# zhen6618/EPRecon

Hardware: AMD Instinct MI355X
Metric: fragments_per_sec (higher is better)
Workload: dtype f32

## Files before the change

### eprecon_amd/_lib.py

```python
import ctypes
import os

import torch

_HERE = os.path.dirname(os.path.abspath(__file__))
LIB_PATH = os.environ.get("EPRECON_LIB_PATH") or os.path.join(_HERE, "libeprecon_hip.so")

_c = ctypes
_vp, _i, _i64, _f, _sz = _c.c_void_p, _c.c_int, _c.c_int64, _c.c_float, _c.c_size_t

SIGNATURES = {
    "eprecon_abi_version": (_i, []),
    "eprecon_build_arch": (_c.c_char_p, []),
    "eprecon_back_project_workspace_bytes": (_sz, [_i64, _i, _i, _i, _i, _i, _i]),
    "eprecon_back_project_async": (_i, [_vp, _i64, _vp, _i, _f, _vp, _i, _vp, _i, _i, _i, _i, _i, _i,
                                        _vp, _vp, _vp, _vp, _vp, _vp, _vp, _vp, _sz, _vp]),
    "eprecon_back_project": (_i, [_vp, _i64, _vp, _i, _f, _vp, _i, _vp, _i, _i, _i, _i, _i, _i, _i,
                                  _vp, _vp, _vp, _vp, _vp, _vp, _vp, _vp, _vp, _sz, _vp]),
    "eprecon_profile_gather_kernel": (_c.c_char_p, []),
    "eprecon_hash_capacity": (_c.c_uint32, [_i64]),
    "eprecon_hash_table_bytes": (_sz, [_c.c_uint32]),
    "eprecon_hash_build_async": (_i, [_vp, _i64, _i, _vp, _c.c_uint32, _vp]),
    "eprecon_hash_build_dn_async": (_i, [_vp, _i64, _vp, _i, _vp, _c.c_uint32, _vp]),
    "eprecon_hash_query_async": (_i, [_vp, _c.c_uint32, _vp, _i64, _i, _vp, _vp]),
    "eprecon_hash_status": (_i, [_vp, _vp]),
    "eprecon_unique_workspace_bytes": (_sz, [_i64]),
    "eprecon_unique_coords_async": (_i, [_vp, _i64, _i, _vp, _c.c_uint32, _vp, _vp, _vp, _vp, _sz, _vp]),
    "eprecon_unique_coords_dn_async": (_i, [_vp, _i64, _vp, _i, _vp, _c.c_uint32, _vp, _vp, _vp, _vp, _sz, _vp]),
    "eprecon_unique_hierarchy_dn_async": (_i, [_vp, _i64, _vp, _i, _vp, _vp, _vp, _vp, _vp, _vp, _sz, _vp]),
    "eprecon_point_quantize_dn_async": (_i, [_vp, _i64, _vp, _f, _vp, _vp, _vp]),
    "eprecon_spvcnn_points_dn_async": (_i, [_vp, _i64, _vp, _i, _i, _vp, _i, _f, _vp, _f, _vp, _vp, _vp, _vp, _vp, _vp]),
    "eprecon_gru_stage_capacity": (_i64, [_vp, _i64, _i]),
    "eprecon_gru_stage_workspace_bytes": (_sz, [_i64]),
    "eprecon_gru_stage_begin_async": (_i, [_vp, _vp]),
    "eprecon_gru_stage_commit_async": (_i, [_vp, _vp, _vp, _vp]),
    "eprecon_kernel_map_async": (_i, [_vp, _c.c_uint32, _vp, _i64, _i, _i, _vp, _vp]),
    "eprecon_kernel_map_self_async": (_i, [_vp, _c.c_uint32, _vp, _i64, _i, _vp, _vp]),
    "eprecon_transpose_map_async": (_i, [_vp, _i64, _vp, _i, _vp, _vp]),
    "eprecon_sparse_conv_async": (_i, [_vp, _i64, _i, _vp, _i, _i64, _vp, _i, _i, _vp, _vp, _i, _i, _i, _vp]),
    "eprecon_conv_bn_partial_bytes": (_sz, [_i64, _i]),
    "eprecon_sparse_conv_fused_async": (_i, [_vp, _i64, _i, _vp, _i, _i64, _vp, _i, _i, _vp, _vp, _i, _vp, _i, _i, _i,
                                             _vp, _vp]),
    "eprecon_conv_desc_async": (_i, [_vp, _vp]),
    "eprecon_exclusive_scan_async": (_i, [_vp, _i64, _vp, _vp, _vp, _vp]),
    "eprecon_conv_desc_partial_rows": (_i64, [_vp]),
    "eprecon_bn_acc_words": (_sz, [_i]),
    "eprecon_conv_desc_takes_bn_acc": (_i, [_vp]),
    "eprecon_batchnorm_acc_affine_async": (_i, [_vp, _i, _i, _i, _f, _vp, _vp, _vp]),
    "eprecon_affine_rows_acc_async": (_i, [_vp, _i64, _i, _i, _vp, _i, _i, _f, _i, _vp, _i, _vp]),
    "eprecon_affine_rows_res_async": (_i, [_vp, _i64, _i, _i, _vp, _vp, _vp, _i, _i, _vp, _i, _vp]),
    "eprecon_batchnorm_finalize_affine_async": (_i, [_vp, _i64, _i, _vp, _vp, _f, _vp, _vp, _vp]),
    "eprecon_affine_rows_async": (_i, [_vp, _i64, _i, _i, _vp, _vp, _i, _vp, _i, _vp]),
    "eprecon_pixel_map_async": (_i, [_i, _i, _i, _i, _vp, _vp]),
    "eprecon_batchnorm_apply_workspace_bytes": (_sz, [_i]),
    "eprecon_batchnorm_apply_partials_async": (_i, [_vp, _i64, _i, _i, _vp, _i64, _vp, _vp, _f, _vp, _i, _i, _vp, _i,
                                                    _vp, _vp, _vp, _sz, _vp]),
    "eprecon_batchnorm_apply_partials_res_async": (_i, [_vp, _i64, _i, _i, _vp, _i64, _vp, _vp, _f, _vp, _i, _vp, _vp, _i, _vp,
                                                        _i, _vp, _sz, _vp]),
    "eprecon_batchnorm_workspace_bytes": (_sz, [_i64, _i]),
    "eprecon_batchnorm_train_async": (_i, [_vp, _i64, _i, _i, _vp, _vp, _f, _vp, _i, _i, _vp, _i, _vp, _vp,
                                           _vp, _sz, _vp]),
    "eprecon_rowwise_layernorm_async": (_i, [_vp, _i64, _i, _i, _vp, _i, _vp, _vp, _f, _i, _i, _vp, _i, _vp]),
    "eprecon_init_select_workspace_bytes": (_sz, [_i, _i]),
    "eprecon_init_select_async": (_i, [_vp, _vp, _i64, _f, _i, _i, _i, _vp, _vp, _vp, _sz, _vp]),
    "eprecon_upsample_async": (_i, [_vp, _i, _vp, _i64, _i, _i, _vp, _vp, _vp]),
    "eprecon_aligned_coords_async": (_i, [_vp, _i64, _vp, _i, _f, _vp, _vp, _vp]),
    "eprecon_point_quantize_async": (_i, [_vp, _i64, _f, _vp, _vp, _vp]),
    "eprecon_segment_workspace_bytes": (_sz, [_i64, _i64]),
    "eprecon_segment_lists_async": (_i, [_vp, _i64, _i64, _vp, _vp, _vp, _sz, _vp]),
    "eprecon_segment_mean_async": (_i, [_vp, _i, _vp, _vp, _i64, _i, _vp, _i, _vp]),
    "eprecon_sphash_async": (_i, [_vp, _i64, _vp, _vp]),
    "eprecon_sphash_order_workspace_bytes": (_sz, [_i64]),
    "eprecon_sphash_order_async": (_i, [_vp, _i64, _vp, _vp, _vp, _sz, _vp]),
    "eprecon_remap_index_async": (_i, [_vp, _i64, _vp, _vp, _i64, _vp, _vp]),
    "eprecon_trilinear_map_async": (_i, [_vp, _c.c_uint32, _vp, _i64, _i, _vp, _vp, _vp]),
    "eprecon_devoxelize_async": (_i, [_vp, _i, _vp, _vp, _i64, _i, _vp, _i, _i, _vp]),
    "eprecon_sparse_conv_wgrad_workspace_bytes": (_sz, [_i, _i64, _i, _i]),
    "eprecon_sparse_conv_wgrad_async": (_i, [_vp, _i, _vp, _i, _vp, _i, _i64, _i, _i, _vp, _vp, _sz, _vp]),
    "eprecon_invert_map_async": (_i, [_vp, _i, _i64, _i64, _vp, _vp]),
    "eprecon_devoxelize_backward_async": (_i, [_vp, _i, _vp, _vp, _i64, _i, _i64, _vp, _i, _vp]),
    "eprecon_gather_rows_scaled_async": (_i, [_vp, _i, _vp, _vp, _i64, _i, _vp, _i, _vp]),
    "eprecon_back_project_backward_async": (_i, [_vp, _i64, _vp, _i, _f, _vp, _vp, _i, _i, _i, _i, _i, _vp, _i, _vp, _vp, _vp]),
    "eprecon_back_project_backward_workspace_bytes": (_sz, [_i, _i, _i, _i, _i]),
    "eprecon_back_project_backward_det_async": (_i, [_vp, _i64, _vp, _i, _f, _vp, _vp, _i, _i, _i, _i, _i, _vp, _i, _vp, _vp, _vp, _sz,
                                                     _vp]),
    "eprecon_devoxelize_backward_csr_async": (_i, [_vp, _i, _vp, _vp, _vp, _i64, _i, _vp, _i, _vp]),
    "eprecon_devoxelize_gate_async": (_i, [_vp, _i, _vp, _vp, _i64, _i, _vp, _i, _i, _vp, _i, _vp, _i, _vp, _i, _vp]),
    "eprecon_devoxelize_gate_tail_async": (_i, [_vp, _i, _vp, _vp, _i64, _i, _vp, _i, _i, _vp, _i, _vp, _i, _vp, _i, _vp, _i, _vp, _i,
                                                _i, _vp]),
    "eprecon_fbv_union_workspace_bytes": (_sz, [_i]),
    "eprecon_fbv_union_async": (_i, [_vp, _vp, _i64, _i, _vp, _vp, _i64, _i, _i, _i, _i, _i, _vp, _vp, _vp, _vp, _vp,
                                     _vp, _vp, _sz, _vp]),
    "eprecon_map_set_fragment": (_i, [_vp, _i]),
    "eprecon_map_stamps_async": (_i, [_vp, _vp, _vp, _i, _c.c_int32, _vp]),
    "eprecon_map_select_boundary_async": (_i, [_vp, _vp, _i, _i, _i, _vp, _vp]),
    "eprecon_map_pack_boundary_async": (_i, [_vp, _vp, _i64, _vp]),
    "eprecon_map_merge_boundary": (_i, [_vp, _vp, _i64, _vp, _i, _vp, _vp]),
    "eprecon_map_create": (_i, [_i, _c.POINTER(_vp)]),
    "eprecon_map_destroy": (_i, [_vp]),
    "eprecon_map_reset": (_i, [_vp]),
    "eprecon_map_size": (_i64, [_vp]),
    "eprecon_map_channels": (_i, [_vp]),
    "eprecon_map_export_async": (_i, [_vp, _vp, _vp, _vp]),
    "eprecon_map_import_async": (_i, [_vp, _vp, _vp, _i64, _vp]),
    "eprecon_map_crop_union": (_i, [_vp, _vp, _vp, _i64, _i, _i, _i, _i, _vp, _vp, _vp, _vp, _vp, _vp]),
    "eprecon_map_gather_async": (_i, [_vp, _vp, _i64, _i, _i, _f, _vp, _i, _vp]),
    "eprecon_map_update_async": (_i, [_vp, _vp, _i64, _vp, _i, _vp]),
    "eprecon_map_target_fuse": (_i, [_vp, _vp, _vp, _i, _vp, _vp, _i64, _vp, _vp]),
    "eprecon_gather_rows_async": (_i, [_vp, _i, _vp, _i64, _i, _f, _vp, _i, _vp]),
    "eprecon_tsdf_integrate_async": (_i, [_vp, _vp, _vp, _vp, _f, _vp, _i, _i, _i, _vp, _vp, _f, _f, _i, _vp, _vp]),
    "eprecon_marching_cubes_table": (_i, [_vp]),
    "eprecon_marching_cubes_workspace_bytes": (_sz, [_i, _i, _i]),
    "eprecon_marching_cubes_count": (_i, [_vp, _i, _i, _i, _f, _vp, _vp, _sz, _vp]),
    "eprecon_marching_cubes_emit_async": (_i, [_vp, _i, _i, _i, _f, _vp, _vp, _vp, _vp, _vp, _vp, _vp, _vp, _vp]),
    "eprecon_marching_cubes_count_masked": (_i, [_vp, _vp, _i, _i, _i, _f, _vp, _vp, _sz, _vp]),
    "eprecon_marching_cubes_emit_masked_async": (_i, [_vp, _vp, _i, _i, _i, _f, _vp, _vp, _vp, _vp, _vp, _vp, _vp, _vp, _vp]),
    "eprecon_render_depth_workspace_bytes": (_sz, [_i64]),
    "eprecon_render_depth_async": (_i, [_vp, _i64, _vp, _i64, _vp, _i, _i, _i, _f, _f, _f, _i, _vp, _i64, _vp, _sz, _vp]),
    "eprecon_depth_metrics_workspace_bytes": (_sz, [_i]),
    "eprecon_depth_metrics_async": (_i, [_vp, _vp, _i, _i64, _vp, _vp, _sz, _vp]),
    "eprecon_point_bounds_async": (_i, [_vp, _i64, _vp, _vp, _vp]),
    "eprecon_voxel_down_sample_workspace_bytes": (_sz, [_i64, _i64]),
    "eprecon_voxel_down_sample": (_i, [_vp, _i64, _vp, _c.c_double, _vp, _vp, _vp, _i64, _vp, _sz, _vp]),
    "eprecon_nn_search_workspace_bytes": (_sz, [_i64, _i64]),
    "eprecon_nn_search_async": (_i, [_vp, _i64, _vp, _i64, _vp, _c.c_double, _vp, _vp, _vp, _vp, _sz, _vp]),
    "eprecon_nearest_voxel_async": (_i, [_vp, _c.c_uint32, _vp, _i64, _vp, _i64, _i, _vp, _vp]),
    "eprecon_upsample2x_nhwc_async": (_i, [_vp, _vp, _i, _i, _i, _i, _vp]),
    "eprecon_decoder_keys_async": (_i, [_vp, _i, _vp, _i, _vp, _vp, _vp, _i64, _i, _vp, _vp, _vp]),
    "eprecon_decoder_query_side_async": (_i, [_vp, _vp]),
    "eprecon_panoptic_stats_async": (_i, [_vp, _i64, _vp, _vp, _i, _i64, _vp, _vp, _vp, _vp]),
    "eprecon_panoptic_assign_async": (_i, [_vp, _vp, _vp, _i64, _vp, _vp]),
    "eprecon_masked_attention_workspace_bytes": (_sz, [_i64, _i, _i, _i]),
    "eprecon_masked_attention_async": (_i, [_vp, _i, _i, _vp, _i, _vp, _i, _i64, _vp, _i, _vp, _i64, _i, _i, _i, _f, _vp, _vp, _sz, _vp]),
    "eprecon_profile_enable": (_i, [_i]),
    "eprecon_profile_gather_ms": (_f, []),
    "eprecon_profile_conv_arm": (_i, [_i, _i, _i, _i64]),
    "eprecon_profile_conv_ms": (_f, [_c.POINTER(_i64), _c.POINTER(_c.c_char_p)]),
    "eprecon_profile_conv_pairs": (_i64, []),
    "eprecon_mlp4x_supported": (_i, [_i, _i]),
    "eprecon_spvcnn_forward_workspace_bytes": (_sz, [_vp]),
    "eprecon_spvcnn_forward_async": (_i, [_vp, _vp]),
# ... 14 lines not shown
    "eprecon_sparsify_workspace_bytes": (_sz, [_i64]),
    "eprecon_sparsify_async": (_i, [_vp, _i, _f, _vp, _vp, _vp, _i, _vp, _i, _i, _i, _i64, _i, _vp, _vp, _vp, _vp, _vp, _vp, _vp,
                                    _sz, _vp]),
    "eprecon_grid_rank_async": (_i, [_vp, _i64, _i, _i, _i, _i, _vp, _vp]),
    "eprecon_conv_pack_weight_floats": (_sz, [_i, _i, _i]),
    "eprecon_conv_pack_weight_async": (_i, [_vp, _i, _i, _i, _vp, _vp]),
    "eprecon_conv_pack_weight16_floats": (_sz, [_i, _i, _i]),
    "eprecon_conv_pack_weight16_async": (_i, [_vp, _i, _i, _i, _vp, _vp]),
    "eprecon_conv_pack_many_async": (_i, [_vp, _i, _vp]),
    "eprecon_nchw_to_nhwc_async": (_i, [_vp, _vp, _i, _i, _i, _vp]),
    "eprecon_views_to_rows_async": (_i, [_vp, _vp]),
}

EPRECON_OK, EPRECON_EMPTY = 0, 1
ABI_VERSION = 1


class EpreconError(RuntimeError):
    pass


_lib = None


def load():
    global _lib
    if _lib is not None:
        return _lib
    if not os.path.exists(LIB_PATH):
        raise EpreconError(
            f"{LIB_PATH} not found: build it with `python -m eprecon_amd.build` "
            "(hipcc --offload-arch=gfx950). eprecon_amd has no CPU fallback.")
    lib = ctypes.CDLL(LIB_PATH)
    for name, (res, args) in SIGNATURES.items():
        fn = getattr(lib, name)
        fn.restype = res
        fn.argtypes = args
    if lib.eprecon_abi_version() != ABI_VERSION:
        raise EpreconError("libeprecon_hip.so ABI version mismatch; rebuild")
    _lib = lib
    return lib


def check(rc, what):
    if rc == EPRECON_OK:
        return True
    if rc == EPRECON_EMPTY:
        return False
    if rc <= -1000:
        raise EpreconError(f"{what}: HIP error {-(rc + 1000)}")
    raise EpreconError(f"{what}: error {rc} "
                       "(-1 bad argument, -2 workspace too small, -3 unsupported size)")


def ptr(t):
    return None if t is None else t.data_ptr()


_raw_stream = getattr(torch._C, "_cuda_getCurrentRawStream", None)
_raw_device = getattr(torch._C, "_cuda_getDevice", None)


def current_stream():
    if _raw_stream is not None and _raw_device is not None:
        return _raw_stream(_raw_device()) or None
    return torch.cuda.current_stream().cuda_stream or None


class ViewsDesc(ctypes.Structure):
    _fields_ = [("src", (ctypes.c_void_p * 16) * 3), ("dst", ctypes.c_void_p * 3), ("channels", ctypes.c_int32 * 3),
                ("hw", ctypes.c_int32 * 3), ("levels", ctypes.c_int32), ("n_views", ctypes.c_int32)]


class ConvDesc(ctypes.Structure):
    _fields_ = [("x", ctypes.c_void_p), ("n_in", ctypes.c_int64), ("ld_x", ctypes.c_int),
                ("nbr", ctypes.c_void_p), ("kvol", ctypes.c_int), ("n_out", ctypes.c_int64),
                ("weight", ctypes.c_void_p), ("cin", ctypes.c_int), ("cout", ctypes.c_int),
                ("bias", ctypes.c_void_p),
                ("residual", ctypes.c_void_p), ("ld_res", ctypes.c_int),
                ("out", ctypes.c_void_p), ("ld_out", ctypes.c_int),
                ("relu", ctypes.c_int), ("accumulate", ctypes.c_int),
                ("in_scale", ctypes.c_void_p), ("in_shift", ctypes.c_void_p), ("in_relu", ctypes.c_int),
                ("res_scale", ctypes.c_void_p), ("res_shift", ctypes.c_void_p), ("res_relu", ctypes.c_int),
                ("bn_partial", ctypes.c_void_p),
                ("ln", ctypes.c_int), ("ln_gamma", ctypes.c_void_p), ("ln_beta", ctypes.c_void_p),
                ("ln_eps", ctypes.c_float), ("ln_post_relu", ctypes.c_int),
                ("img_h", ctypes.c_int), ("img_w", ctypes.c_int), ("img_maps", ctypes.c_int),
                ("vox_rank", ctypes.c_void_p), ("grid_x", ctypes.c_int), ("grid_y", ctypes.c_int), ("grid_z", ctypes.c_int),
                ("packed_weight", ctypes.c_void_p), ("packed_weight16", ctypes.c_void_p),
                ("workspace", ctypes.c_void_p), ("workspace_bytes", ctypes.c_size_t),
                ("bn_acc", ctypes.c_void_p), ("bn_acc_ld", ctypes.c_int), ("bn_acc_c0", ctypes.c_int),
                ("bn_gamma", ctypes.c_void_p), ("bn_beta", ctypes.c_void_p),
                ("in_acc", ctypes.c_void_p), ("in_acc_ld", ctypes.c_int), ("in_acc_c0", ctypes.c_int),
                ("in_eps", ctypes.c_float), ("in_affine_scratch", ctypes.c_void_p)]


class GruStageDesc(ctypes.Structure):
    _fields_ = [("map", ctypes.c_void_p), ("target_map", ctypes.c_void_p),
                ("cur_coords", ctypes.c_void_p), ("cur_feat", ctypes.c_void_p), ("n_cur", ctypes.c_int64), ("ld_cur", ctypes.c_int),
                ("dim", ctypes.c_int), ("interval", ctypes.c_int), ("activity_mode", ctypes.c_int),
                ("rel", ctypes.c_int32 * 3),
                ("tsdf_gt", ctypes.c_void_p), ("occ_gt", ctypes.c_void_p),
                ("origin", ctypes.c_void_p), ("w2ac", ctypes.c_void_p),
                ("voxel_size", ctypes.c_float), ("resolution", ctypes.c_float),
                ("ch_voxel", ctypes.c_int), ("batch_index", ctypes.c_int),
                ("capacity", ctypes.c_int64),
                ("updated", ctypes.c_void_p), ("out_coords", ctypes.c_void_p), ("r_coords", ctypes.c_void_p),
                ("hx_voxel", ctypes.c_void_p), ("hx_image", ctypes.c_void_p), ("tsdf_target", ctypes.c_void_p),
                ("scaled1", ctypes.c_void_p), ("vox1", ctypes.c_void_p), ("inverse1", ctypes.c_void_p), ("uniq1", ctypes.c_void_p),
                ("table1", ctypes.c_void_p),
                ("scaled2", ctypes.c_void_p), ("vox2", ctypes.c_void_p), ("inverse2", ctypes.c_void_p), ("uniq2", ctypes.c_void_p),
                ("table2", ctypes.c_void_p),
                ("table_capacity", ctypes.c_uint32),
                ("counts", ctypes.c_void_p),
                ("workspace", ctypes.c_void_p), ("workspace_bytes", ctypes.c_size_t)]


class DecoderLayerDesc(ctypes.Structure):
    _PTRS_A = ["o_attn", "state_in", "query_pos", "cross_out_wt", "cross_out_b", "cross_ln_g", "cross_ln_b", "self_in_wt", "self_in_b",
               "self_out_wt", "self_out_b", "self_ln_g", "self_ln_b", "ffn1_wt", "ffn1_b", "ffn2_wt", "ffn2_b", "ffn_ln_g", "ffn_ln_b",
               "dec_ln_g", "dec_ln_b", "cls_wt", "cls_b", "m1_wt", "m1_b", "m2_wt", "m2_b", "m3_wt", "m3_b", "next_q_wt", "next_q_b"]
    _PTRS_B = ["state_out", "cls_out", "mask_embed_out", "next_q_out", "workspace"]
    _fields_ = ([(n, ctypes.c_int) for n in ("n_queries", "channels", "n_heads", "ffn_dim", "n_class_logits", "mask_hidden")]
                + [(n, ctypes.c_void_p) for n in _PTRS_A] + [("ln_eps", ctypes.c_float)] + [(n, ctypes.c_void_p) for n in _PTRS_B])


class GruFinishDesc(ctypes.Structure):
    _fields_ = ([(n, ctypes.c_int64) for n in ("n", "m1", "m2")]
                + [(n, ctypes.c_void_p) for n in ("inverse1", "inverse2", "uniq1", "uniq2", "table1", "table2")]
                + [("table_capacity", ctypes.c_uint32)] + [(n, ctypes.c_void_p) for n in ("scaled1", "scaled2")]
                + [("literal", ctypes.c_int)]
                + [(n, ctypes.c_void_p) for n in ("offsets1", "order1", "offsets2", "order2", "nbr1", "nbr2", "idx8_1", "weight8_1",
                                                  "idx8_2", "weight8_2", "perm1", "rank1", "perm2", "rank2", "workspace")]
                + [("workspace_bytes", ctypes.c_size_t)])


class SpvcnnGeometryDesc(ctypes.Structure):
    _fields_ = ([(n, ctypes.c_int64) for n in ("n", "n1", "n2", "n4")]
                + [(n, ctypes.c_void_p) for n in ("scaled", "vox", "inverse1", "coords1", "coords2", "coords4", "parent2", "parent4",
                                                  "table1", "table2", "table4")]
                + [(n, ctypes.c_uint32) for n in ("capacity1", "capacity2", "capacity4")]
                + [(n, ctypes.c_void_p) for n in ("offsets1", "order1", "idx4", "offsets4", "order4", "down12", "up21", "down24", "up42",
                                                  "k1", "k2", "k4", "idx8_1", "weight8_1", "idx8_4", "weight8_4", "workspace")]
                + [("workspace_bytes", ctypes.c_size_t)])


SPVCNN_CONVS = 27


class SpvcnnConv(ctypes.Structure):
    _fields_ = [(n, ctypes.c_void_p) for n in ("weight", "packed_weight", "packed_weight16")] + [(n, ctypes.c_int) for n in ("kvol", "cin", "cout")]


class SpvcnnBn(ctypes.Structure):
    _fields_ = [("gamma", ctypes.c_void_p), ("beta", ctypes.c_void_p), ("eps", ctypes.c_float)]


class SpvcnnForwardDesc(ctypes.Structure):
    _fields_ = ([(n, ctypes.c_int64) for n in ("n", "n1", "n2", "n4")] + [("cin", ctypes.c_int), ("cs", ctypes.c_int * 5)]
                + [("feat", ctypes.c_void_p), ("ld_feat", ctypes.c_int)]
                + [(n, ctypes.c_void_p) for n in ("offsets1", "order1", "offsets4", "order4", "k1", "k2", "k4", "down12", "up21", "down24",
                                                  "up42", "idx8_1", "weight8_1", "idx8_4", "weight8_4")]
                + [("conv", SpvcnnConv * SPVCNN_CONVS), ("bn", SpvcnnBn * SPVCNN_CONVS)]
                + [("out", ctypes.c_void_p), ("ld_out", ctypes.c_int), ("workspace", ctypes.c_void_p), ("workspace_bytes", ctypes.c_size_t)])


class Mlp4xHead(ctypes.Structure):
# ... 129 lines not shown
```

### eprecon_amd/csrc/conv_common.hpp

```cpp
#pragma once
#include "common.hpp"

namespace epconv {

struct ConvParams {
    const float *x;
    const int32_t *nbr;
    const float *w;
    const float *bias;
    float *out;
    int n_out, K, Cin, Cout, ld_x, ld_out;
    int64_t x_bytes;
    int relu;
    int accumulate;
    const float *res;
    int ld_res;
    float *bn_partial;
    const float *in_scale, *in_shift;
    int in_relu;
    const float *res_scale, *res_shift;
    int res_relu;
    int ln;
    const float *ln_gamma, *ln_beta;
    float ln_eps;
    int ln_post_relu;
    int img_h, img_w, img_maps;
    int flex_partial;
    const int32_t *vox_rank;
    int gx, gy, gz;
    const float *wq;
    const float *wq16;
    int debug;
    int splitk_pipe;
    void *ws;
    size_t ws_bytes;
    long long *bn_acc;
    int bn_acc_ld, bn_acc_c0;
    const float *bn_gamma, *bn_beta;
    const long long *in_acc;
    int in_acc_ld, in_acc_c0;
    float in_eps;
};

constexpr int kBnCopies = 8, kBnWords = 7;
#ifndef EP_BN_ABL
#define EP_BN_ABL 0
#endif

__device__ __forceinline__ void bn_limbs(double x, long long &l0, long long &l1, long long &l2)
{
    const double v = x * 1099511627776.0;
    const double hi = floor(v * (1.0 / 1099511627776.0));
    l0 = (long long)(v - hi * 1099511627776.0);
    const long long h = (long long)hi;
    l1 = h & ((1ll << 40) - 1);
    l2 = h >> 40;
}

__device__ __forceinline__ void bn_acc_add(long long *acc, int ld, int c, int copy, float n, float mean, float m2)
{
    if (n <= 0.0f || (EP_BN_ABL & 1)) return;
    unsigned long long *a = reinterpret_cast<unsigned long long *>(acc) + ((size_t)copy * ld + c) * kBnWords;
    const double dn = (double)n, dm = (double)mean;
    long long l0, l1, l2;
    bn_limbs(dn * dm, l0, l1, l2);
    atomicAdd(a + 0, (unsigned long long)l0);
    if (EP_BN_ABL & 4) return;
    atomicAdd(a + 1, (unsigned long long)l1); atomicAdd(a + 2, (unsigned long long)l2);
    bn_limbs((double)m2 + dn * dm * dm, l0, l1, l2);
    atomicAdd(a + 3, (unsigned long long)l0); atomicAdd(a + 4, (unsigned long long)l1); atomicAdd(a + 5, (unsigned long long)l2);
    atomicAdd(a + 6, (unsigned long long)(long long)n);
}

__device__ __forceinline__ void bn_acc_affine(const long long *acc, int ld, int c, float eps, float &scale, float &shift)
{
    if (EP_BN_ABL & 2) { scale = 1.0f; shift = 0.0f; return; }
    long long w[kBnWords] = {0, 0, 0, 0, 0, 0, 0};
#pragma unroll 1
    for (int k = 0; k < kBnCopies; ++k) {
        const long long *a = acc + ((size_t)k * ld + c) * kBnWords;
#pragma unroll
        for (int j = 0; j < kBnWords; ++j) w[j] += a[j];
    }
    const double two40 = 1099511627776.0;
    const double s1 = ((double)w[2] * two40 + (double)w[1]) + (double)w[0] * (1.0 / two40);
    const double s2 = ((double)w[5] * two40 + (double)w[4]) + (double)w[3] * (1.0 / two40);
    const double n = (double)w[6];
    const float *gb = reinterpret_cast<const float *>(acc + (size_t)kBnCopies * ld * kBnWords);
    const double mean = n > 0.0 ? s1 / n : 0.0;
    double var = n > 0.0 ? s2 / n - mean * mean : 0.0;
    if (var < 0.0) var = 0.0;
    const float sc = gb[c] / sqrtf((float)var + eps);
    scale = sc;
    shift = gb[ld + c] - (float)mean * sc;
}

template <int THREADS, bool ACC = true>
__device__ __forceinline__ void stage_in_affine(const ConvParams &p, float *sAff, int cpad, int tid)
{
    if (!p.in_scale) return;
    for (int c = tid; c < cpad; c += THREADS) {
        float sc = 0.0f, sh = 0.0f;
        if (c < p.Cin) {
            if (ACC && p.in_acc) bn_acc_affine(p.in_acc, p.in_acc_ld, p.in_acc_c0 + c, p.in_eps, sc, sh);
            else { sc = p.in_scale[c]; sh = p.in_shift[c]; }
        }
        sAff[c] = sc;
        sAff[cpad + c] = sh;
    }
}

__device__ __forceinline__ void bn_acc_publish(const ConvParams &p, int col, int copy, bool first, float n, float mean, float m2)
{
    bn_acc_add(p.bn_acc, p.bn_acc_ld, p.bn_acc_c0 + col, copy & (kBnCopies - 1), n, mean, m2);
    if (first) {
        float *gb = reinterpret_cast<float *>(p.bn_acc + (size_t)kBnCopies * p.bn_acc_ld * kBnWords);
        gb[p.bn_acc_c0 + col] = p.bn_gamma ? p.bn_gamma[col] : 1.0f;
        gb[p.bn_acc_ld + p.bn_acc_c0 + col] = p.bn_beta ? p.bn_beta[col] : 0.0f;
    }
}

constexpr int kWaves = 4;
typedef float f32x4 __attribute__((ext_vector_type(4)));
typedef unsigned int u32x4 __attribute__((ext_vector_type(4)));

__device__ __forceinline__ void chan_merge(float &n_a, float &mean_a, float &m2_a, float n_b, float mean_b, float m2_b)
{
    if (n_b == 0.0f) return;
    if (n_a == 0.0f) {
        n_a = n_b; mean_a = mean_b; m2_a = m2_b;
        return;
    }
    const float n = n_a + n_b;
    const float d = mean_b - mean_a;
    mean_a = mean_a + d * (n_b / n);
    m2_a = m2_a + m2_b + d * d * (n_a * n_b / n);
    n_a = n;
}

template <int CT, bool ACC = false>
__device__ __forceinline__ void tile16_epilogue(const ConvParams &p, const f32x4 (&acc)[CT], const int (&orow)[4], float *sStat,
                                                int partial_row)
{
    const int tid = threadIdx.x;
    const int lane = tid & 63, wave = tid >> 6;
    const int l16 = lane & 15, q = lane >> 4;
    float v[CT][4];
    bool colok[CT];
#pragma unroll
    for (int t = 0; t < CT; ++t) {
        const int col = 16 * t + l16;
        colok[t] = col < p.Cout;
        const float b = (p.bias && colok[t]) ? p.bias[col] : 0.0f;
        const float rs = (p.res_scale && colok[t]) ? p.res_scale[col] : 1.0f;
        const float rb = (p.res_scale && colok[t]) ? p.res_shift[col] : 0.0f;
#pragma unroll
        for (int j = 0; j < 4; ++j) {
            float val = 0.0f;
            if (colok[t] && orow[j] >= 0) {
                val = acc[t][j] + b;
                if (p.relu) val = fmaxf(val, 0.0f);
                if (p.res) {
                    float rv = p.res[(size_t)orow[j] * p.ld_res + col];
                    if (p.res_scale) {
                        rv = fmaf(rv, rs, rb);
                        if (p.res_relu) rv = fmaxf(rv, 0.0f);
                    }
                    val += rv;
                }
            }
            v[t][j] = val;
        }
    }
    if (p.ln) {
        const float inv_c = 1.0f / (float)p.Cout;
#pragma unroll
        for (int j = 0; j < 4; ++j) {
            float sum = 0.0f;
#pragma unroll
            for (int t = 0; t < CT; ++t) sum += v[t][j];
#pragma unroll
            for (int m = 8; m > 0; m >>= 1) sum += __shfl_xor(sum, m);
            const float mean = sum * inv_c;
            float sq = 0.0f;
#pragma unroll
            for (int t = 0; t < CT; ++t) {
                const float d = colok[t] ? v[t][j] - mean : 0.0f;
                v[t][j] = d;
                sq = fmaf(d, d, sq);
            }
#pragma unroll
            for (int m = 8; m > 0; m >>= 1) sq += __shfl_xor(sq, m);
            const float inv = 1.0f / sqrtf(sq * inv_c + p.ln_eps);
#pragma unroll
            for (int t = 0; t < CT; ++t) {
                const int col = 16 * t + l16;
                float y = fmaf(v[t][j] * inv, (p.ln_gamma && colok[t]) ? p.ln_gamma[col] : 1.0f, (p.ln_beta && colok[t]) ? p.ln_beta[col] : 0.0f);
                if (p.ln_post_relu) y = fmaxf(y, 0.0f);
                v[t][j] = y;
            }
        }
    }
#pragma unroll
    for (int t = 0; t < CT; ++t)
#pragma unroll
        for (int j = 0; j < 4; ++j)
            if (colok[t] && orow[j] >= 0) p.out[(size_t)orow[j] * p.ld_out + 16 * t + l16] = v[t][j];
    if (p.bn_partial || (ACC && p.bn_acc)) {
#pragma unroll
        for (int t = 0; t < CT; ++t) {
            float n = 0.0f, sum = 0.0f;
#pragma unroll
            for (int j = 0; j < 4; ++j)
                if (orow[j] >= 0) { n += 1.0f; sum += v[t][j]; }
            float mean = n > 0.0f ? sum / n : 0.0f, m2 = 0.0f;
#pragma unroll
            for (int j = 0; j < 4; ++j)
                if (orow[j] >= 0) { const float d = v[t][j] - mean; m2 = fmaf(d, d, m2); }
#pragma unroll
            for (int m = 16; m < 64; m <<= 1) {
                const float on = __shfl_xor(n, m), om = __shfl_xor(mean, m), oq = __shfl_xor(m2, m);
                const bool lower = (lane & m) == 0;
                float a_n = lower ? n : on, a_mean = lower ? mean : om, a_m2 = lower ? m2 : oq;
                chan_merge(a_n, a_mean, a_m2, lower ? on : n, lower ? om : mean, lower ? oq : m2);
                n = a_n; mean = a_mean; m2 = a_m2;
            }
            if (q == 0) {
                float *d = sStat + (wave * 3) * 16 * CT + 16 * t + l16;
                d[0] = n; d[16 * CT] = mean; d[2 * 16 * CT] = m2;
            }
        }
        __syncthreads();
        if (tid < 16 * CT && tid < p.Cout) {
            float a_n = 0.0f, a_mean = 0.0f, a_m2 = 0.0f;
#pragma unroll
            for (int w = 0; w < kWaves; ++w)
                chan_merge(a_n, a_mean, a_m2, sStat[(w * 3) * 16 * CT + tid], sStat[(w * 3 + 1) * 16 * CT + tid], sStat[(w * 3 + 2) * 16 * CT + tid]);
            if (p.bn_partial) {
                float *dst = p.bn_partial + (size_t)partial_row * 3 * p.Cout + tid;
                dst[0] = a_n; dst[p.Cout] = a_mean; dst[2 * p.Cout] = a_m2;
            }
            if (ACC && p.bn_acc) bn_acc_publish(p, tid, partial_row, partial_row == 0, a_n, a_mean, a_m2);
        }
    }
}

bool direct16_ok(const ConvParams &p);
constexpr int kDirectRows = 128;
int launch_direct16(const ConvParams &p, hipStream_t st);
int direct16_partial_block_rows(const ConvParams &p);

bool tile2d16_ok(const ConvParams &p);
int64_t tile2d16_partial_rows(const ConvParams &p);
int launch_tile2d16(const ConvParams &p, hipStream_t st);


}
```

### eprecon_amd/csrc/norm.hip

```cpp
#include <stdlib.h>

#include "common.hpp"
#include "conv_common.hpp"

namespace {
using namespace ep;

constexpr int kBnPerThread = 8;

__device__ __forceinline__ void chan_merge(float &n_a, float &mean_a, float &m2_a, float n_b, float mean_b, float m2_b)
{
    if (n_b == 0.0f) return;
    if (n_a == 0.0f) {
        n_a = n_b; mean_a = mean_b; m2_a = m2_b;
        return;
    }
    const float n = n_a + n_b;
    const float d = mean_b - mean_a;
    mean_a = mean_a + d * (n_b / n);
    m2_a = m2_a + m2_b + d * d * (n_a * n_b / n);
    n_a = n;
}

__global__ __launch_bounds__(256) void bn_stats_kernel(const float *x, int n, int C, int ld, float *partial)
{
    __shared__ float sN[256], sMean[256], sM2[256];
    const int tid = threadIdx.x;
    const int rpi = 256 / C;
    const int col = tid % C, rsub = tid / C;
    const bool active = rsub < rpi;
    const int r0 = blockIdx.x * (kBnPerThread * rpi);
    float v[kBnPerThread];
    float cnt = 0.0f, sum = 0.0f;
#pragma unroll
    for (int k = 0; k < kBnPerThread; ++k) {
        const int r = r0 + k * rpi + rsub;
        const bool ok = active && r < n;
        v[k] = ok ? x[(size_t)r * ld + col] : 0.0f;
        cnt += ok ? 1.0f : 0.0f;
        sum += v[k];
    }
    const float mean = cnt > 0.0f ? sum / cnt : 0.0f;
    float m2 = 0.0f;
#pragma unroll
    for (int k = 0; k < kBnPerThread; ++k) {
        const int r = r0 + k * rpi + rsub;
        if (active && r < n) {
            const float d = v[k] - mean;
            m2 = fmaf(d, d, m2);
        }
    }
    sN[tid] = cnt; sMean[tid] = mean; sM2[tid] = m2;
    __syncthreads();
    for (int s = 1; s < rpi; s <<= 1) {
        if (active && (rsub % (2 * s)) == 0 && rsub + s < rpi) {
            float n = sN[tid], m = sMean[tid], q = sM2[tid];
            const int o = tid + s * C;
            chan_merge(n, m, q, sN[o], sMean[o], sM2[o]);
            sN[tid] = n; sMean[tid] = m; sM2[tid] = q;
        }
        __syncthreads();
    }
    if (tid < C) {
        float *p = partial + (size_t)blockIdx.x * 3 * C;
        p[tid] = sN[tid]; p[C + tid] = sMean[tid]; p[2 * C + tid] = sM2[tid];
    }
}

__global__ __launch_bounds__(256) void bn_finalize_kernel(const float *partial, int nblk, int C, float *mean_out,
                                                          float *var_out)
{
    __shared__ float sN[256], sMean[256], sM2[256];
    const int c = blockIdx.x, tid = threadIdx.x;
    float a_n = 0.0f, a_mean = 0.0f, a_m2 = 0.0f;
    for (int b = tid; b < nblk; b += 4 * 256) {
        float vn[4], vm[4], vq[4];
#pragma unroll
        for (int u = 0; u < 4; ++u) {
            const int bb = b + u * 256;
            const float *p = partial + (size_t)(bb < nblk ? bb : b) * 3 * C;
            vn[u] = bb < nblk ? p[c] : 0.0f;
            vm[u] = p[C + c];
            vq[u] = p[2 * C + c];
        }
#pragma unroll
        for (int u = 0; u < 4; ++u) chan_merge(a_n, a_mean, a_m2, vn[u], vm[u], vq[u]);
    }
    sN[tid] = a_n; sMean[tid] = a_mean; sM2[tid] = a_m2;
    __syncthreads();
    for (int s = 128; s > 0; s >>= 1) {
        if (tid < s) {
            float n = sN[tid], m = sMean[tid], q = sM2[tid];
            chan_merge(n, m, q, sN[tid + s], sMean[tid + s], sM2[tid + s]);
            sN[tid] = n; sMean[tid] = m; sM2[tid] = q;
        }
        __syncthreads();
    }
    if (tid == 0) {
        mean_out[c] = sMean[0];
        var_out[c] = sN[0] > 0.0f ? sM2[0] / sN[0] : 0.0f;
    }
}

__global__ __launch_bounds__(256) void bn_finalize_affine_kernel(const float *partial, int nblk, int C, const float *gamma,
                                                                 const float *beta, float eps, float *scale_out,
                                                                 float *shift_out)
{
    __shared__ float sN[4], sMean[4], sM2[4];
    const int c = blockIdx.x, tid = threadIdx.x;
    const float g_c = gamma ? gamma[c] : 1.0f, b_c = beta ? beta[c] : 0.0f;
    float a_n = 0.0f, a_mean = 0.0f, a_m2 = 0.0f;
    for (int b = tid; b < nblk; b += 4 * 256) {
        float vn[4], vm[4], vq[4];
#pragma unroll
        for (int u = 0; u < 4; ++u) {
            const int bb = b + u * 256;
            const float *p = partial + (size_t)(bb < nblk ? bb : b) * 3 * C;
            vn[u] = bb < nblk ? p[c] : 0.0f;
            vm[u] = p[C + c];
            vq[u] = p[2 * C + c];
        }
#pragma unroll
        for (int u = 0; u < 4; ++u) chan_merge(a_n, a_mean, a_m2, vn[u], vm[u], vq[u]);
    }
    const int lane = tid & 63;
#pragma unroll
    for (int m = 1; m < 64; m <<= 1) {
        const float on = __shfl_xor(a_n, m), om = __shfl_xor(a_mean, m), oq = __shfl_xor(a_m2, m);
        float ln = (lane & m) ? on : a_n, lm = (lane & m) ? om : a_mean, lq = (lane & m) ? oq : a_m2;
        chan_merge(ln, lm, lq, (lane & m) ? a_n : on, (lane & m) ? a_mean : om, (lane & m) ? a_m2 : oq);
        a_n = ln; a_mean = lm; a_m2 = lq;
    }
    if (lane == 0) { sN[tid >> 6] = a_n; sMean[tid >> 6] = a_mean; sM2[tid >> 6] = a_m2; }
    __syncthreads();
    if (tid == 0) {
        float n = sN[0], mean = sMean[0], m2 = sM2[0];
        for (int w = 1; w < 4; ++w) chan_merge(n, mean, m2, sN[w], sMean[w], sM2[w]);
        const float var = n > 0.0f ? m2 / n : 0.0f;
        const float sc = g_c / sqrtf(var + eps);
        scale_out[c] = sc;
        shift_out[c] = b_c - mean * sc;
    }
}

__global__ __launch_bounds__(256) void bn_apply_kernel(const float *x, int n, int C, int ld_x,
                                                       const float *mean, const float *var,
                                                       const float *gamma, const float *beta, float eps,
                                                       const float *res, int ld_res, const float *res_scale,
                                                       const float *res_shift, int relu, float *out, int ld_out)
{
    const size_t e = (size_t)blockIdx.x * 256 + threadIdx.x;
    if (e >= (size_t)n * C) return;
    const int r = (int)(e / C), c = (int)(e - (size_t)r * C);
    const float inv = 1.0f / sqrtf(var[c] + eps);
    float v = (x[(size_t)r * ld_x + c] - mean[c]) * inv;
    v = v * (gamma ? gamma[c] : 1.0f) + (beta ? beta[c] : 0.0f);
    if (res) {
        float rv = res[(size_t)r * ld_res + c];
        if (res_scale) rv = fmaf(rv, res_scale[c], res_shift[c]);
        v += rv;
    }
    if (relu) v = fmaxf(v, 0.0f);
    out[(size_t)r * ld_out + c] = v;
}

__global__ __launch_bounds__(256) void rowwise_ln_kernel(const float *x, int n, int C, int ld_x,
                                                         const float *res, int ld_res,
                                                         const float *gamma, const float *beta, float eps,
                                                         int pre_relu, int post_relu, float *out,
                                                         int ld_out)
{
    const int g = threadIdx.x & 7;
    const int r = blockIdx.x * 32 + (threadIdx.x >> 3);
    const bool live = r < n;
    const float *xr = x + (size_t)(live ? r : 0) * ld_x;
    const float *rr = res ? res + (size_t)(live ? r : 0) * ld_res : nullptr;
    auto value = [&](int c) -> float {
        float v = xr[c];
        if (pre_relu) v = fmaxf(v, 0.0f);
        if (rr) v += rr[c];
        return v;
    };
    float s = 0.0f;
    if (live)
        for (int c = g; c < C; c += 8) s += value(c);
    s += __shfl_xor(s, 1);
    s += __shfl_xor(s, 2);
    s += __shfl_xor(s, 4);
    const float mean = s / (float)C;
    float q = 0.0f;
    if (live)
        for (int c = g; c < C; c += 8) {
            const float d = value(c) - mean;
            q = fmaf(d, d, q);
        }
    q += __shfl_xor(q, 1);
    q += __shfl_xor(q, 2);
    q += __shfl_xor(q, 4);
    const float inv = 1.0f / sqrtf(q / (float)C + eps);
    if (live)
        for (int c = g; c < C; c += 8) {
            float v = (value(c) - mean) * inv * (gamma ? gamma[c] : 1.0f) + (beta ? beta[c] : 0.0f);
            if (post_relu) v = fmaxf(v, 0.0f);
            out[(size_t)r * ld_out + c] = v;
        }
}

__global__ __launch_bounds__(256) void affine_rows_kernel(const float *x, int n, int C, int ld_x, const float *scale,
                                                          const float *shift, int relu, float *out, int ld_out)
{
    const size_t e = (size_t)blockIdx.x * 256 + threadIdx.x;
    if (e >= (size_t)n * C) return;
    const int r = (int)(e / C), c = (int)(e - (size_t)r * C);
    float v = fmaf(x[(size_t)r * ld_x + c], scale[c], shift[c]);
    if (relu) v = fmaxf(v, 0.0f);
    out[(size_t)r * ld_out + c] = v;
}

__global__ __launch_bounds__(256) void bn_acc_affine_kernel(const long long *acc, int ld, int c0, int C, float eps, float *scale,
                                                            float *shift)
{
    const int c = blockIdx.x * 256 + threadIdx.x;
    if (c >= C) return;
    float sc, sh;
    epconv::bn_acc_affine(acc, ld, c0 + c, eps, sc, sh);
    scale[c] = sc;
    shift[c] = sh;
}

constexpr int kAccRowsMaxC = 512;
__global__ __launch_bounds__(256) void affine_rows_acc_kernel(const float *x, int n, int C, int ld_x, const long long *acc, int ld,
                                                              int c0, float eps, int relu, float *out, int ld_out)
{
    __shared__ float sAff[2 * kAccRowsMaxC];
    for (int c = threadIdx.x; c < C; c += 256) epconv::bn_acc_affine(acc, ld, c0 + c, eps, sAff[c], sAff[kAccRowsMaxC + c]);
    __syncthreads();
    for (int k = 0; k < 16; ++k) {
        const size_t e = ((size_t)blockIdx.x * 16 + k) * 256 + threadIdx.x;
        if (e >= (size_t)n * C) return;
        const int r = (int)(e / C), c = (int)(e - (size_t)r * C);
        float v = fmaf(x[(size_t)r * ld_x + c], sAff[c], sAff[kAccRowsMaxC + c]);
        if (relu) v = fmaxf(v, 0.0f);
        out[(size_t)r * ld_out + c] = v;
    }
}

__global__ __launch_bounds__(256) void affine_rows_res_kernel(const float *x, int n, int C, int ld_x, const float *scale,
                                                              const float *shift, const float *res, int ld_res, int relu,
                                                              float *out, int ld_out)
{
    const size_t e = (size_t)blockIdx.x * 256 + threadIdx.x;
    if (e >= (size_t)n * C) return;
    const int r = (int)(e / C), c = (int)(e - (size_t)r * C);
    float v = fmaf(x[(size_t)r * ld_x + c], scale[c], shift[c]);
    if (res) v += res[(size_t)r * ld_res + c];
    if (relu) v = fmaxf(v, 0.0f);
    out[(size_t)r * ld_out + c] = v;
}

int bn_finalize_apply(const float *x, int64_t n, int channels, int ld_x, const float *partial, int nblk,
                      const float *gamma, const float *beta, float eps, const float *residual, int ld_res,
                      int relu, float *out, int ld_out, float *mean, float *var, hipStream_t st,
                      const float *res_scale = nullptr, const float *res_shift = nullptr)
{
    hipLaunchKernelGGL(bn_finalize_kernel, dim3(channels), dim3(256), 0, st, partial, nblk, channels, mean, var);
    EP_LAUNCH_CHECK();
    const size_t total = (size_t)n * channels;
    hipLaunchKernelGGL(bn_apply_kernel, dim3((unsigned)ceil_div((int64_t)total, 256)), dim3(256), 0, st, x,
                       (int)n, channels, ld_x, (const float *)mean, (const float *)var, gamma, beta, eps,
                       residual, ld_res, res_scale, res_shift, relu, out, ld_out);
    EP_LAUNCH_CHECK();
    return EPRECON_OK;
}

}

extern "C" {

static inline int bn_rows_per_block(int channels) { return kBnPerThread * (256 / channels); }

size_t eprecon_batchnorm_workspace_bytes(int64_t n, int channels)
{
    if (channels <= 0 || channels > 256) return 0;
    const size_t nblk = (size_t)ceil_div(n > 0 ? n : 1, bn_rows_per_block(channels));
    return align_up(nblk * 3 * channels * sizeof(float), 256) + 2 * align_up((size_t)channels * sizeof(float), 256);
}

int eprecon_batchnorm_train_async(const float *x, int64_t n, int channels, int ld_x, const float *gamma,
                                  const float *beta, float eps, const float *residual, int ld_res,
                                  int relu, float *out, int ld_out, float *mean_out, float *var_out,
                                  void *workspace, size_t workspace_bytes, void *stream)
{
    if (!x || !out || n < 0 || channels <= 0 || channels > 256 || ld_x < channels || ld_out < channels ||
        !workspace)
        return EPRECON_ERR_ARG;
    if (workspace_bytes < eprecon_batchnorm_workspace_bytes(n, channels)) return EPRECON_ERR_WORKSPACE;
    if (n == 0) return EPRECON_OK;
    hipStream_t st = (hipStream_t)stream;
    const int nblk = (int)ceil_div(n, bn_rows_per_block(channels));
    char *ws = reinterpret_cast<char *>(workspace);
    float *partial = reinterpret_cast<float *>(ws);
    ws += align_up((size_t)nblk * 3 * channels * sizeof(float), 256);
    float *mean = mean_out ? mean_out : reinterpret_cast<float *>(ws);
    ws += align_up((size_t)channels * sizeof(float), 256);
    float *var = var_out ? var_out : reinterpret_cast<float *>(ws);
    hipLaunchKernelGGL(bn_stats_kernel, dim3(nblk), dim3(256), 0, st, x, (int)n, channels, ld_x, partial);
    EP_LAUNCH_CHECK();
    return bn_finalize_apply(x, n, channels, ld_x, partial, nblk, gamma, beta, eps, residual, ld_res, relu, out,
                             ld_out, mean, var, st);
}

size_t eprecon_batchnorm_apply_workspace_bytes(int channels)
{
    return 2 * align_up((size_t)(channels > 0 ? channels : 1) * sizeof(float), 256);
}

int eprecon_batchnorm_apply_partials_async(const float *x, int64_t n, int channels, int ld_x,
                                           const float *partial, int64_t nblk, const float *gamma,
                                           const float *beta, float eps, const float *residual,
                                           int ld_res, int relu, float *out, int ld_out, float *mean_out,
                                           float *var_out, void *workspace, size_t workspace_bytes,
                                           void *stream)
{
    if (!x || !out || !partial || n < 0 || nblk <= 0 || nblk > 0x7fffffff || channels <= 0 || ld_x < channels ||
        ld_out < channels || !workspace)
        return EPRECON_ERR_ARG;
    if (workspace_bytes < eprecon_batchnorm_apply_workspace_bytes(channels)) return EPRECON_ERR_WORKSPACE;
    if (n == 0) return EPRECON_OK;
    char *ws = reinterpret_cast<char *>(workspace);
    float *mean = mean_out ? mean_out : reinterpret_cast<float *>(ws);
    ws += align_up((size_t)channels * sizeof(float), 256);
    float *var = var_out ? var_out : reinterpret_cast<float *>(ws);
    return bn_finalize_apply(x, n, channels, ld_x, partial, (int)nblk, gamma, beta, eps, residual, ld_res, relu,
                             out, ld_out, mean, var, (hipStream_t)stream);
}

int eprecon_batchnorm_apply_partials_res_async(const float *x, int64_t n, int channels, int ld_x, const float *partial,
                                               int64_t nblk, const float *gamma, const float *beta, float eps,
                                               const float *residual, int ld_res, const float *res_scale,
                                               const float *res_shift, int relu, float *out, int ld_out, void *workspace,
                                               size_t workspace_bytes, void *stream)
{
    if (!x || !out || !partial || !residual || !res_scale || !res_shift || n < 0 || nblk <= 0 || nblk > 0x7fffffff ||
        channels <= 0 || ld_x < channels || ld_out < channels || ld_res < channels || !workspace)
        return EPRECON_ERR_ARG;
    if (workspace_bytes < eprecon_batchnorm_apply_workspace_bytes(channels)) return EPRECON_ERR_WORKSPACE;
    if (n == 0) return EPRECON_OK;
    char *ws = reinterpret_cast<char *>(workspace);
    float *mean = reinterpret_cast<float *>(ws);
    float *var = reinterpret_cast<float *>(ws + align_up((size_t)channels * sizeof(float), 256));
    return bn_finalize_apply(x, n, channels, ld_x, partial, (int)nblk, gamma, beta, eps, residual, ld_res, relu, out, ld_out,
                             mean, var, (hipStream_t)stream, res_scale, res_shift);
}

int eprecon_batchnorm_finalize_affine_async(const float *partial, int64_t nblk, int channels, const float *gamma,
                                            const float *beta, float eps, float *scale_out, float *shift_out,
                                            void *stream)
{
    if (!partial || !scale_out || !shift_out || nblk <= 0 || nblk > 0x7fffffff || channels <= 0) return EPRECON_ERR_ARG;
    hipLaunchKernelGGL(bn_finalize_affine_kernel, dim3(channels), dim3(256), 0, (hipStream_t)stream, partial, (int)nblk,
                       channels, gamma, beta, eps, scale_out, shift_out);
    EP_LAUNCH_CHECK();
    return EPRECON_OK;
}

int eprecon_affine_rows_async(const float *x, int64_t n, int channels, int ld_x, const float *scale,
                              const float *shift, int relu, float *out, int ld_out, void *stream)
{
    if (!x || !out || !scale || !shift || n < 0 || channels <= 0 || ld_x < channels || ld_out < channels ||
        n * channels > 0x7fffffffll * 256)
        return EPRECON_ERR_ARG;
    if (n == 0) return EPRECON_OK;
    hipLaunchKernelGGL(affine_rows_kernel, dim3((unsigned)ceil_div(n * channels, (int64_t)256)), dim3(256), 0,
                       (hipStream_t)stream, x, (int)n, channels, ld_x, scale, shift, relu, out, ld_out);
    EP_LAUNCH_CHECK();
    return EPRECON_OK;
}

int eprecon_batchnorm_acc_affine_async(const long long *acc, int acc_ld, int acc_c0, int channels, float eps, float *scale_out,
                                       float *shift_out, void *stream)
{
    if (!acc || !scale_out || !shift_out || channels <= 0 || acc_c0 < 0 || acc_c0 + channels > acc_ld) return EPRECON_ERR_ARG;
    hipLaunchKernelGGL(bn_acc_affine_kernel, dim3((unsigned)ceil_div(channels, 256)), dim3(256), 0, (hipStream_t)stream, acc, acc_ld,
                       acc_c0, channels, eps, scale_out, shift_out);
    EP_LAUNCH_CHECK();
    return EPRECON_OK;
}

int eprecon_affine_rows_acc_async(const float *x, int64_t n, int channels, int ld_x, const long long *acc, int acc_ld, int acc_c0,
                                  float eps, int relu, float *out, int ld_out, void *stream)
{
    if (!x || !out || !acc || n < 0 || channels <= 0 || channels > kAccRowsMaxC || ld_x < channels || ld_out < channels ||
        acc_c0 < 0 || acc_c0 + channels > acc_ld || n * channels > 0x7fffffffll * 256)
        return EPRECON_ERR_ARG;
    if (n == 0) return EPRECON_OK;
    hipLaunchKernelGGL(affine_rows_acc_kernel, dim3((unsigned)ceil_div(n * channels, (int64_t)4096)), dim3(256), 0,
                       (hipStream_t)stream, x, (int)n, channels, ld_x, acc, acc_ld, acc_c0, eps, relu, out, ld_out);
    EP_LAUNCH_CHECK();
    return EPRECON_OK;
}

int eprecon_affine_rows_res_async(const float *x, int64_t n, int channels, int ld_x, const float *scale,
                                  const float *shift, const float *residual, int ld_res, int relu, float *out,
                                  int ld_out, void *stream)
{
    if (!x || !out || !scale || !shift || n < 0 || channels <= 0 || ld_x < channels || ld_out < channels ||
        (residual && ld_res < channels) || n * channels > 0x7fffffffll * 256)
        return EPRECON_ERR_ARG;
    if (n == 0) return EPRECON_OK;
    hipLaunchKernelGGL(affine_rows_res_kernel, dim3((unsigned)ceil_div(n * channels, (int64_t)256)), dim3(256), 0,
                       (hipStream_t)stream, x, (int)n, channels, ld_x, scale, shift, residual, ld_res, relu, out, ld_out);
    EP_LAUNCH_CHECK();
    return EPRECON_OK;
}

int eprecon_rowwise_layernorm_async(const float *x, int64_t n, int channels, int ld_x,
                                    const float *residual, int ld_res, const float *gamma,
                                    const float *beta, float eps, int pre_relu, int post_relu,
                                    float *out, int ld_out, void *stream)
{
    if (!x || !out || n < 0 || channels <= 0 || ld_x < channels || ld_out < channels) return EPRECON_ERR_ARG;
    if (n == 0) return EPRECON_OK;
    hipLaunchKernelGGL(rowwise_ln_kernel, dim3((unsigned)ceil_div(n, 32)), dim3(256), 0,
                       (hipStream_t)stream, x, (int)n, channels, ld_x, residual, ld_res, gamma, beta, eps,
                       pre_relu, post_relu, out, ld_out);
    EP_LAUNCH_CHECK();
    return EPRECON_OK;
}

}
```

### eprecon_amd/csrc/sparse_conv.hip

```cpp
#include <stdio.h>
#include <stdlib.h>
#include <string.h>

#include "common.hpp"
#include "conv_common.hpp"

namespace {
using namespace ep;
using namespace epconv;

typedef float f32x16 __attribute__((ext_vector_type(16)));


template <int TN>
__device__ __forceinline__ void stage_weights(float *dst, const float *w, int row0, int row_end, int stride,
                                              int ncols, int rows, int tid)
{
    const int total = rows * TN;
    if (stride == TN && ncols >= TN && (reinterpret_cast<uintptr_t>(w) & 15) == 0) {
        const float4 *src = reinterpret_cast<const float4 *>(w + (size_t)row0 * stride);
        float4 *d4 = reinterpret_cast<float4 *>(dst);
        const int valid4 = max(0, min(rows, row_end - row0)) * (TN / 4);
#pragma unroll 4
        for (int e = tid; e < total / 4; e += 256) d4[e] = e < valid4 ? src[min(e, max(valid4 - 1, 0))] : make_float4(0.f, 0.f, 0.f, 0.f);
// ... 93 lines not shown
        const float inv = 1.0f / sqrtf(q * inv_c + p.ln_eps);
        const int row = rm((r & 3) + 8 * (r >> 2) + 4 * half);
#pragma unroll
        for (int t = 0; t < NT; ++t) {
            float y = fmaf(acc[t][r] * inv, gam[t], bet[t]);
            if (p.ln_post_relu) y = fmaxf(y, 0.0f);
            if (colok[t] && row >= 0) p.out[(size_t)row * p.ld_out + t * 32 + r32] = y;
        }
    }
}

template <int NT, bool ACC = true, class RowMap>
__device__ __forceinline__ void conv_epilogue(const ConvParams &p, f32x16 (&acc)[NT], RowMap rm, int col0, int r32,
                                              int half, int wave, float *sStat, int partial_row, int ncb)
{
    constexpr int TN = 32 * NT;
    if (p.ln) {
        conv_epilogue_ln<NT>(p, acc, rm, r32, half);
        return;
    }
    const bool stats = p.bn_partial != nullptr || (ACC && p.bn_acc != nullptr);
    if (stats) __syncthreads();
#pragma unroll
    for (int t = 0; t < NT; ++t) {
        const int col = col0 + t * 32 + r32;
        const bool colok = col < p.Cout;
        const float b = (p.bias && colok) ? p.bias[col] : 0.0f;
        const float rs = (p.res_scale && colok) ? p.res_scale[col] : 1.0f;
        const float rb = (p.res_scale && colok) ? p.res_shift[col] : 0.0f;
        float vals[16];
        float cnt = 0.0f, sum = 0.0f;
#pragma unroll
        for (int r = 0; r < 16; ++r) {
            const int row = rm((r & 3) + 8 * (r >> 2) + 4 * half);
            float v = 0.0f;
            if (colok && row >= 0) {
                float *o = p.out + (size_t)row * p.ld_out + col;
                v = acc[t][r] + b;
                if (p.accumulate) v += *o;
                if (p.relu) v = fmaxf(v, 0.0f);
                if (p.res) {
                    float rv = p.res[(size_t)row * p.ld_res + col];
                    if (p.res_scale) {
                        rv = fmaf(rv, rs, rb);
                        if (p.res_relu) rv = fmaxf(rv, 0.0f);
                    }
                    v += rv;
                }
                *o = v;
                cnt += 1.0f;
            }
            vals[r] = v;
            sum += v;
        }
        if (stats) {
            float mean = cnt > 0.0f ? sum / cnt : 0.0f;
            float m2 = 0.0f;
#pragma unroll
            for (int r = 0; r < 16; ++r) {
                const int row = rm((r & 3) + 8 * (r >> 2) + 4 * half);
                if (row >= 0) {
                    const float d = vals[r] - mean;
                    m2 = fmaf(d, d, m2);
                }
            }
            const float on = __shfl_xor(cnt, 32), omean = __shfl_xor(mean, 32), om2 = __shfl_xor(m2, 32);
            float a_n = half ? on : cnt, a_mean = half ? omean : mean, a_m2 = half ? om2 : m2;
            chan_merge(a_n, a_mean, a_m2, half ? cnt : on, half ? mean : omean, half ? m2 : om2);
            if (half == 0) {
                float *d = sStat + (wave * 3) * TN + t * 32 + r32;
                d[0] = a_n; d[TN] = a_mean; d[2 * TN] = a_m2;
            }
        }
    }
    if (stats) {
        __syncthreads();
        const int tid = threadIdx.x;
        if (tid < TN && col0 + tid < p.Cout) {
            float a_n = 0.0f, a_mean = 0.0f, a_m2 = 0.0f;
#pragma unroll
            for (int w = 0; w < kWaves; ++w)
                chan_merge(a_n, a_mean, a_m2, sStat[(w * 3) * TN + tid], sStat[(w * 3 + 1) * TN + tid],
                           sStat[(w * 3 + 2) * TN + tid]);
            if (!ACC || p.bn_partial) {
                float *dst = p.bn_partial + (size_t)partial_row * 3 * p.Cout + col0 + tid;
                dst[0] = a_n; dst[p.Cout] = a_mean; dst[2 * p.Cout] = a_m2;
            }
            if (ACC && p.bn_acc) bn_acc_publish(p, col0 + tid, partial_row, partial_row == 0, a_n, a_mean, a_m2);
        }
    }
}

template <int NT, bool VEC4>
__global__ __launch_bounds__(256) void spconv_mfma_kernel(ConvParams p)
{
    extern __shared__ __attribute__((aligned(16))) char smem[];
    constexpr int TN = 32 * NT;
    float *sW = reinterpret_cast<float *>(smem);
    int *sNbr = reinterpret_cast<int *>(sW + 2 * kSlabC * TN);
    int *sActive = sNbr + p.K * kRowsPerBlock;
    const int cinA = (p.Cin + 3) & ~3;
    float *sAff = reinterpret_cast<float *>(sActive + ((p.K + 3) & ~3));

    const int tid = threadIdx.x;
    const int lane = tid & 63, wave = tid >> 6;
    const int r32 = lane & 31, half = lane >> 5;
    const int row0 = blockIdx.x * kRowsPerBlock;
    const int col0 = blockIdx.y * TN;

    for (int k = tid; k < p.K; k += 256) sActive[k] = 0;
    stage_in_affine<256>(p, sAff, cinA, tid);
    __syncthreads();
    for (int e = tid; e < p.K * kRowsPerBlock; e += 256) {
        const int k = e / kRowsPerBlock, r = e - k * kRowsPerBlock;
        const int row = row0 + r;
        int j = -1;
        if (row < p.n_out) j = p.nbr ? p.nbr[(size_t)k * p.n_out + row] : row;
        sNbr[e] = j;
        if (j >= 0) sActive[k] = 1;
    }
    __syncthreads();

    f32x16 acc[NT];
#pragma unroll
    for (int t = 0; t < NT; ++t)
#pragma unroll
        for (int r = 0; r < 16; ++r) acc[t][r] = 0.0f;

    const int nslab = (p.Cin + kSlabC - 1) / kSlabC;
    int buf = 0;
    bool have_prev = false;
    for (int k = 0; k < p.K; ++k) {
        if (!sActive[k]) continue;
        const int j = sNbr[k * kRowsPerBlock + wave * kRowsPerWave + r32];
        const float *xrow = p.x + (size_t)(j >= 0 ? j : 0) * p.ld_x;
        const float *wk = p.w + (size_t)k * p.Cin * p.Cout + col0;
        for (int sl = 0; sl < nslab; ++sl) {
            const int c0 = sl * kSlabC;
            float *dstW = sW + buf * kSlabC * TN;
            stage_weights<TN>(dstW, wk, c0, p.Cin, p.Cout, p.Cout - col0, kSlabC, tid);
            float a[4][4];
#pragma unroll
            for (int ch = 0; ch < 4; ++ch) {
                const int c = c0 + ch * 8 + 4 * half;
                if (VEC4) {
                    float4 v = make_float4(0.f, 0.f, 0.f, 0.f);
                    if (j >= 0 && c < p.Cin) v = *reinterpret_cast<const float4 *>(xrow + c);
                    if (p.Cin & 3) {
                        if (c + 1 >= p.Cin) v.y = 0.0f;
                        if (c + 2 >= p.Cin) v.z = 0.0f;
                        if (c + 3 >= p.Cin) v.w = 0.0f;
                    }
                    a[ch][0] = v.x; a[ch][1] = v.y; a[ch][2] = v.z; a[ch][3] = v.w;
                } else {
#pragma unroll
                    for (int s = 0; s < 4; ++s) a[ch][s] = (j >= 0 && c + s < p.Cin) ? xrow[c + s] : 0.0f;
                }
            }
            __syncthreads();
            (void)have_prev;
            const float *srcW = sW + buf * kSlabC * TN;
            const int nch = min(4, (p.Cin - c0 + 7) / 8);
            if (p.in_scale) {
#pragma unroll
                for (int ch = 0; ch < 4; ++ch) {
                    const int c = c0 + ch * 8 + 4 * half;
#pragma unroll
                    for (int s = 0; s < 4; ++s) {
                        const bool ok = j >= 0 && c + s < p.Cin;
                        float v = fmaf(a[ch][s], sAff[min(c + s, cinA - 1)], sAff[cinA + min(c + s, cinA - 1)]);
// ... 498 lines not shown
    const int v = tid % (32 * WV);
    const int own = d3_rank(sX, (((v >> 5) + 1) * kD3HY + ((v >> 3) & 3) + 1) * kD3HZ + (v & 7) + 1, P, cin_pad);
    return __syncthreads_or(own >= 0) != 0;
}

template <int NCH, int WV, int THREADS = 64 * WV>
__device__ __forceinline__ void d3_stage_rows(const ConvParams &p, float *sX, int tid, int dbg, int cbase)
{
    constexpr int cin_pad = NCH * 8, P = cin_pad + 4, C4 = cin_pad / 4;
    constexpr int kThreads = THREADS, kD3Halo = d3_halo(WV);
    constexpr int kItems = kD3Halo * C4;
    constexpr int kIter = (kItems + kThreads - 1) / kThreads;
    float4 hv[kIter];
    int hr[kIter];
    const int last4 = ((p.Cin + 3) & ~3) - 4;
    constexpr bool kFixedGroup = kThreads % C4 == 0;
    float4 sc0 = make_float4(1.f, 1.f, 1.f, 1.f), sh0 = make_float4(0.f, 0.f, 0.f, 0.f);
    if (kFixedGroup && p.in_scale) {
        sc0 = *reinterpret_cast<const float4 *>(p.in_scale + min(cbase + (tid % C4) * 4, last4));
        sh0 = *reinterpret_cast<const float4 *>(p.in_shift + min(cbase + (tid % C4) * 4, last4));
    }
#pragma unroll
    for (int it = 0; it < kIter; ++it) {
        const int e = min(tid + it * kThreads, kItems - 1);
        const int cell = e / C4, c4 = e - cell * C4;
        hr[it] = d3_rank(sX, cell, P, cin_pad);
        if (dbg & 4) hv[it] = make_float4(1.f, 1.f, 1.f, 1.f);
        else hv[it] = *reinterpret_cast<const float4 *>(p.x + (size_t)max(hr[it], 0) * p.ld_x + min(cbase + c4 * 4, last4));
    }
#pragma unroll
    for (int it = 0; it < kIter; ++it) {
        const int e = tid + it * kThreads;
        if (e >= kItems) break;
        const int cell = e / C4, c4 = e - cell * C4;
        const int c = cbase + c4 * 4;
        float4 v4 = hv[it];
        if (p.in_scale) {
            float4 sc = sc0, sh = sh0;
            if (!kFixedGroup) {
                sc = *reinterpret_cast<const float4 *>(p.in_scale + min(c, last4));
                sh = *reinterpret_cast<const float4 *>(p.in_shift + min(c, last4));
            }
            v4.x = fmaf(v4.x, sc.x, sh.x); v4.y = fmaf(v4.y, sc.y, sh.y);
            v4.z = fmaf(v4.z, sc.z, sh.z); v4.w = fmaf(v4.w, sc.w, sh.w);
            if (p.in_relu) {
                v4.x = fmaxf(v4.x, 0.f); v4.y = fmaxf(v4.y, 0.f); v4.z = fmaxf(v4.z, 0.f); v4.w = fmaxf(v4.w, 0.f);
            }
        }
        if (hr[it] < 0 || c >= p.Cin) v4 = make_float4(0.f, 0.f, 0.f, 0.f);
        *reinterpret_cast<float4 *>(sX + cell * P + c4 * 4) = v4;
    }
    __syncthreads();
}

template <int NCH, int WV, int THREADS = 64 * WV>
__device__ __forceinline__ bool d3_stage_halo(const ConvParams &p, int x0, int y0, int z0, float *sX, int tid, int dbg)
{
    if (!d3_stage_ranks<NCH, WV, THREADS>(p, x0, y0, z0, sX, tid)) return false;
    d3_stage_rows<NCH, WV, THREADS>(p, sX, tid, dbg, 0);
    return true;
}

template <int NCH>
__global__ __launch_bounds__(256) void conv3d_tile_narrow_kernel(ConvParams p, int tiles_y, int tiles_z, int ntiles)
{
    constexpr int cin_pad = NCH * 8, P = cin_pad + 4, C4 = cin_pad / 4;
    constexpr int WV = kD3WvNarrow, kD3Halo = d3_halo(WV);
    static_assert(WV == 4, "the cell mapping below covers 128 cells with 256 threads");
    extern __shared__ __attribute__((aligned(16))) char smem[];
    float *sX = reinterpret_cast<float *>(smem);
    float *sWn = sX + kD3Halo * P;
    float *sRed = sWn + 27 * cin_pad;
    const int tid = threadIdx.x;
    const int lane = tid & 63, wave = tid >> 6;
    const int tile = xcd_remap((int)blockIdx.x, (int)gridDim.x);
    if (tile >= ntiles) return;
    int x0, y0, z0;
    d3_tile_origin<WV>(tile, tiles_y, tiles_z, x0, y0, z0);
    for (int e = tid; e < 27 * cin_pad; e += 256) {
        const int k = e / cin_pad, c = e - k * cin_pad;
        sWn[e] = c < p.Cin ? p.w[((size_t)k * p.Cin + c) * p.Cout] : 0.0f;
    }
    if (!d3_stage_halo<NCH, WV>(p, x0, y0, z0, sX, tid, p.debug)) {
        if (p.bn_partial && tid == 0) {
            float *dst = p.bn_partial + (size_t)tile * 3 * p.Cout;
            dst[0] = 0.0f; dst[p.Cout] = 0.0f; dst[2 * p.Cout] = 0.0f;
        }
        return;
    }
    const int v = tid >> 1, part = tid & 1;
    const int cell0 = (((v >> 5) + 1) * kD3HY + ((v >> 3) & 3) + 1) * kD3HZ + (v & 7) + 1;
    const int row = d3_rank(sX, cell0, P, cin_pad);
    float acc = 0.0f;
#pragma unroll
    for (int k = 0; k < 27; ++k) {
        const int dx = k % 3 - 1, dy = (k / 3) % 3 - 1, dz = k / 9 - 1;
        const float *xk = sX + (cell0 + (dx * kD3HY + dy) * kD3HZ + dz) * P;
#pragma unroll
        for (int j = 0; j < C4 / 2; ++j) {
            const int c = (2 * j + part) * 4;
            const float4 a = *reinterpret_cast<const float4 *>(xk + c);
            const float4 w = *reinterpret_cast<const float4 *>(sWn + k * cin_pad + c);
            acc = fmaf(a.x, w.x, acc); acc = fmaf(a.y, w.y, acc); acc = fmaf(a.z, w.z, acc); acc = fmaf(a.w, w.w, acc);
        }
    }
    acc += __shfl_xor(acc, 1);
    float n = 0.0f, mean = 0.0f, m2 = 0.0f;
    if (part == 0 && row >= 0) {
        float *o = p.out + (size_t)row * p.ld_out;
        float val = acc + (p.bias ? p.bias[0] : 0.0f);
        if (p.accumulate) val += *o;
        if (p.relu) val = fmaxf(val, 0.0f);
        if (p.res) {
            float rv = p.res[(size_t)row * p.ld_res];
            if (p.res_scale) {
                rv = fmaf(rv, p.res_scale[0], p.res_shift[0]);
                if (p.res_relu) rv = fmaxf(rv, 0.0f);
            }
            val += rv;
        }
        *o = val;
        n = 1.0f; mean = val;
    }
    if (p.bn_partial) {
#pragma unroll
        for (int m = 1; m < 64; m <<= 1) {
            const float on = __shfl_xor(n, m), omean = __shfl_xor(mean, m), om2 = __shfl_xor(m2, m);
            const bool lower = (lane & m) == 0;
            float a_n = lower ? n : on, a_mean = lower ? mean : omean, a_m2 = lower ? m2 : om2;
            chan_merge(a_n, a_mean, a_m2, lower ? on : n, lower ? omean : mean, lower ? om2 : m2);
            n = a_n; mean = a_mean; m2 = a_m2;
        }
        if (lane == 0) { sRed[wave * 3] = n; sRed[wave * 3 + 1] = mean; sRed[wave * 3 + 2] = m2; }
        __syncthreads();
        if (tid == 0) {
            float a_n = 0.0f, a_mean = 0.0f, a_m2 = 0.0f;
            for (int w = 0; w < kWaves; ++w) chan_merge(a_n, a_mean, a_m2, sRed[w * 3], sRed[w * 3 + 1], sRed[w * 3 + 2]);
            float *dst = p.bn_partial + (size_t)tile * 3 * p.Cout;
            dst[0] = a_n; dst[p.Cout] = a_mean; dst[2 * p.Cout] = a_m2;
        }
    }
}

constexpr int kD16X = 2;
constexpr int kD16Halo = (kD16X + 2) * kD3HY * kD3HZ;

__device__ __forceinline__ void pack_weights16_body(const float *w, int K, int Cin, int Cout, int kch, int ct, float *wq, int first,
                                                    int step)
{
    const int total = K * kch * ct * 256;
    const int rem = Cout - 16 * (ct - 1);
    const int total_tail = (rem >= 1 && rem <= 8) ? K * kch * 128 : 0;
    for (int e = first; e < total_tail; e += step) {
        const int sidx = e & 3, n = (e >> 2) & 3, q = (e >> 4) & 3, cg = (e >> 6) & 1;
        const int r = e >> 7;
        const int kc = r % kch, k = r / kch;
        const bool tail8 = kc == kch - 1 && Cin - 16 * kc <= 8;
        const int c = tail8 ? (sidx < 2 ? 16 * kc + 2 * q + sidx : Cin) : 16 * kc + 4 * q + sidx;
        const int co = 16 * (ct - 1) + 4 * cg + n;
        wq[(size_t)total + e] = (c < Cin && co < Cout) ? w[((size_t)k * Cin + c) * Cout + co] : 0.0f;
    }
    for (int e = first; e < total; e += step) {
        const int sidx = e & 3, col = (e >> 2) & 15, q = (e >> 6) & 3;
        int r = e >> 8;
        const int t = r % ct; r /= ct;
        const int kc = r % kch, k = r / kch;
        const bool tail8 = kc == kch - 1 && Cin - 16 * kc <= 8;
        const int c = tail8 ? (sidx < 2 ? 16 * kc + 2 * q + sidx : Cin) : 16 * kc + 4 * q + sidx;
        const int co = 16 * t + col;
        wq[e] = (c < Cin && co < Cout) ? w[((size_t)k * Cin + c) * Cout + co] : 0.0f;
    }
}
__global__ void pack_weights16_kernel(const float *w, int K, int Cin, int Cout, int kch, int ct, float *wq)
{
    pack_weights16_body(w, K, Cin, Cout, kch, ct, wq, blockIdx.x * blockDim.x + threadIdx.x, gridDim.x * blockDim.x);
}

__global__ void pack_many_kernel(const eprecon_pack_job *jobs)
{
    const eprecon_pack_job j = jobs[blockIdx.y];
    const int first = blockIdx.x * blockDim.x + threadIdx.x, step = gridDim.x * blockDim.x;
    if (j.kind == 0) {
        int nt, ncb;
        d3_columns(j.cout, &nt, &ncb);
        pack_weights_body(j.weight, j.kvol, j.cin, j.cout, (j.cin + 7) / 8, nt, ncb, j.packed, first, step);
    } else {
        pack_weights16_body(j.weight, j.kvol, j.cin, j.cout, (j.cin + 15) / 16, (j.cout + 15) / 16, j.packed, first, step);
    }
}

#ifndef EP_TILE16_MIX
#define EP_TILE16_MIX 1
#endif
template <int CT, int KCH>
__global__ __launch_bounds__(256, 7) void conv3d_tile16_kernel(ConvParams p, int tiles_y, int tiles_z, int ntiles)
{
    constexpr int cin_pad = 16, NCH = 2;
    constexpr int P = cin_pad + 4;
    extern __shared__ __attribute__((aligned(16))) char smem[];
    float *sX = reinterpret_cast<float *>(smem);
    const int tid = threadIdx.x;
    const int lane = tid & 63, wave = tid >> 6;
    const int l16 = lane & 15, q = lane >> 4;
    const int tile = xcd_remap((int)blockIdx.x, (int)gridDim.x);
    if (tile >= ntiles) return;
    int x0, y0, z0;
    d3_tile_origin<kD16X>(tile, tiles_y, tiles_z, x0, y0, z0);
    float *sStat = sX;

    if (!d3_stage_ranks<NCH, kD16X, 256>(p, x0, y0, z0, sX, tid)) {
        if (p.bn_partial && tid < 16 * CT && tid < p.Cout) {
            float *dst = p.bn_partial + (size_t)tile * 3 * p.Cout + tid;
            dst[0] = 0.0f; dst[p.Cout] = 0.0f; dst[2 * p.Cout] = 0.0f;
        }
        return;
    }
    const int wx = wave >> 1, wy = 2 * (wave & 1);
    const int cell_a = ((wx + 1) * kD3HY + wy + (l16 >> 3) + 1) * kD3HZ + (l16 & 7) + 1;
    int orow[4];
#pragma unroll
    for (int j = 0; j < 4; ++j) {
        const int r = 4 * q + j;
        orow[j] = d3_rank(sX, ((wx + 1) * kD3HY + wy + (r >> 3) + 1) * kD3HZ + (r & 7) + 1, P, cin_pad);
    }
    const bool work = __ballot(d3_rank(sX, cell_a, P, cin_pad) >= 0) != 0ull && !(p.debug & 1);

    f32x4 acc[CT];
#pragma unroll
    for (int t = 0; t < CT; ++t) acc[t] = f32x4{0.0f, 0.0f, 0.0f, 0.0f};

    const float *xa = sX + (cell_a - (kD3HY + 1) * kD3HZ - 1) * P + 4 * q;
    constexpr unsigned kStepBytes = CT * 1024u, kOffBytes = KCH * kStepBytes;
    const __amdgpu_buffer_rsrc_t wrsrc =
        __builtin_amdgcn_make_buffer_rsrc(const_cast<float *>(p.wq), 0, (int)(27 * kOffBytes), 0x00020000);
    const unsigned wlane = (unsigned)lane * 16u;
    constexpr int kAheadB = 2;
    for (int pass = 0; pass < KCH; ++pass) {
        if (pass > 0) __syncthreads();
        d3_stage_rows<NCH, kD16X, 256>(p, sX, tid, p.debug, 16 * pass);
        if (!work) continue;
        float4 bq[kAheadB + 1][CT];
        float4 aq[2];
        auto load_b = [&](int k, float4(&dst)[CT]) {
#pragma unroll
            for (int t = 0; t < CT; ++t) {
                const u32x4 v = __builtin_amdgcn_raw_buffer_load_b128(wrsrc, wlane + (unsigned)t * 1024u,
                                                                      (unsigned)((p.debug & 2) ? 0 : k) * kOffBytes + (unsigned)pass * kStepBytes, 0);
                dst[t] = make_float4(__uint_as_float(v.x), __uint_as_float(v.y), __uint_as_float(v.z), __uint_as_float(v.w));
            }
        };
        auto load_a = [&](int k) {
            const int dx = k % 3, dy = (k / 3) % 3, dz = k / 9;
            return *reinterpret_cast<const float4 *>(xa + ((dx * kD3HY + dy) * kD3HZ + dz) * P);
        };
#pragma unroll
        for (int k = 0; k < kAheadB; ++k) load_b(k, bq[k]);
        aq[0] = load_a(0);
#pragma unroll
        for (int k = 0; k < 27; ++k) {
            if (k + kAheadB < 27) load_b(k + kAheadB, bq[(k + kAheadB) % (kAheadB + 1)]);
            if (k + 1 < 27) aq[(k + 1) & 1] = load_a(k + 1);
#if EP_TILE16_MIX == 0
            __builtin_amdgcn_sched_barrier(0);
#endif
            const float4 av = aq[k & 1];
            const float4(&bk)[CT] = bq[k % (kAheadB + 1)];
#pragma unroll
            for (int t = 0; t < CT; ++t) acc[t] = __builtin_amdgcn_mfma_f32_16x16x4f32(av.x, bk[t].x, acc[t], 0, 0, 0);
#pragma unroll
            for (int t = 0; t < CT; ++t) acc[t] = __builtin_amdgcn_mfma_f32_16x16x4f32(av.y, bk[t].y, acc[t], 0, 0, 0);
#pragma unroll
            for (int t = 0; t < CT; ++t) acc[t] = __builtin_amdgcn_mfma_f32_16x16x4f32(av.z, bk[t].z, acc[t], 0, 0, 0);
#pragma unroll
            for (int t = 0; t < CT; ++t) acc[t] = __builtin_amdgcn_mfma_f32_16x16x4f32(av.w, bk[t].w, acc[t], 0, 0, 0);
#if EP_TILE16_MIX == 1
#pragma unroll
            for (int sg = 0; sg < CT; ++sg) {
                __builtin_amdgcn_sched_group_barrier(0x020, 1, 0);
                __builtin_amdgcn_sched_group_barrier(0x008, 4, 0);
            }
            __builtin_amdgcn_sched_group_barrier(0x100, 1, 0);
#endif
            __builtin_amdgcn_sched_barrier(0);
        }
    }
    __syncthreads();

    tile16_epilogue<CT>(p, acc, orow, sStat, tile);
}

enum D3Kind { kD3None = 0, kD3Narrow = 1, kD3Tile16 = 2 };

int d3_tiles_kind(const ConvParams &p, int kind, int *ty = nullptr, int *tz = nullptr)
{
    const int wv = kind == kD3Tile16 ? kD16X : kD3WvNarrow;
    const int tx = (p.gx + wv - 1) / wv, tyy = (p.gy + kD3Y - 1) / kD3Y, tzz = (p.gz + kD3Z - 1) / kD3Z;
    if (ty) *ty = tyy;
// ... 929 lines not shown
}

extern "C" int64_t eprecon_profile_conv_executed_pairs(void)
{
    ConvProf &g = g_conv_prof;
    if (!g.recorded || !g.pairs_dev || hipEventSynchronize(g.stop) != hipSuccess) return -1;
    unsigned long long v = 0;
    if (hipMemcpy(&v, g.pairs_dev + 1, sizeof(v), hipMemcpyDeviceToHost) != hipSuccess) return -1;
    return (int64_t)v;
}

extern "C" size_t eprecon_conv_pack_weight_floats(int kvol, int cin, int cout)
{
    if (kvol <= 0 || cin <= 0 || cout <= 0) return 0;
    int nt, ncb;
    d3_columns(cout, &nt, &ncb);
    return (size_t)ncb * kvol * ((cin + 7) / 8) * 2 * nt * 32 * 4;
}

extern "C" int eprecon_conv_pack_weight_async(const float *weight, int kvol, int cin, int cout, float *packed, void *stream)
{
    if (!weight || !packed || kvol <= 0 || cin <= 0 || cout <= 0) return EPRECON_ERR_ARG;
    int nt, ncb;
    d3_columns(cout, &nt, &ncb);
    const size_t total = eprecon_conv_pack_weight_floats(kvol, cin, cout);
    hipLaunchKernelGGL(pack_weights_kernel, dim3((unsigned)min((size_t)1024, (total + 255) / 256)), dim3(256), 0, (hipStream_t)stream,
                       weight, kvol, cin, cout, (cin + 7) / 8, nt, ncb, packed);
    EP_LAUNCH_CHECK();
    return EPRECON_OK;
}

extern "C" size_t eprecon_conv_pack_weight16_floats(int kvol, int cin, int cout)
{
    if (kvol <= 0 || cin <= 0 || cout <= 0 || cout > 64) return 0;
    const int rem = cout - 16 * ((cout + 15) / 16 - 1);
    return (size_t)kvol * ((cin + 15) / 16) * ((cout + 15) / 16) * 256 + (rem <= 8 ? (size_t)kvol * ((cin + 15) / 16) * 128 : 0);
}

extern "C" int eprecon_conv_pack_weight16_async(const float *weight, int kvol, int cin, int cout, float *packed, void *stream)
{
    if (!weight || !packed || kvol <= 0 || cin <= 0 || cout <= 0 || cout > 64) return EPRECON_ERR_ARG;
    const size_t total = eprecon_conv_pack_weight16_floats(kvol, cin, cout);
    hipLaunchKernelGGL(pack_weights16_kernel, dim3((unsigned)min((size_t)1024, (total + 255) / 256)), dim3(256), 0, (hipStream_t)stream,
                       weight, kvol, cin, cout, (cin + 15) / 16, (cout + 15) / 16, packed);
    EP_LAUNCH_CHECK();
    return EPRECON_OK;
}

extern "C" int eprecon_conv_pack_many_async(const eprecon_pack_job *jobs_dev, int njobs, void *stream)
{
    if (njobs < 0 || (njobs > 0 && !jobs_dev) || njobs > 65535) return EPRECON_ERR_ARG;
    if (njobs == 0) return EPRECON_OK;
    hipLaunchKernelGGL(pack_many_kernel, dim3(32, (unsigned)njobs), dim3(256), 0, (hipStream_t)stream, jobs_dev);
    EP_LAUNCH_CHECK();
    return EPRECON_OK;
}

extern "C" size_t eprecon_conv_bn_partial_bytes(int64_t n_out, int cout)
{
    return (size_t)ep::ceil_div(n_out > 0 ? n_out : 1, (int64_t)128) * 3 * (size_t)(cout > 0 ? cout : 1) * sizeof(float);
}

static int conv_check_and_run(ConvParams &p, int64_t n_in, int64_t n_out, void *stream)
{
    if (!p.x || !p.w || !p.out || n_in < 0 || n_out < 0 || p.K <= 0 || p.K > 64 || p.Cin <= 0 || p.Cout <= 0 ||
        p.ld_x < p.Cin || p.ld_out < p.Cout || (p.res && p.ld_res < p.Cout))
        return EPRECON_ERR_ARG;
    if (!p.nbr && !p.vox_rank && p.K != 1) return EPRECON_ERR_ARG;
    if (!p.nbr && n_in != n_out) return EPRECON_ERR_ARG;
    if ((p.in_scale == nullptr) != (p.in_shift == nullptr) || (p.res_scale == nullptr) != (p.res_shift == nullptr))
        return EPRECON_ERR_ARG;
    if (p.Cout > 4096 || n_out > 0x7fffffff) return EPRECON_ERR_UNSUPPORTED;
    if (n_out == 0) return EPRECON_OK;
    p.n_out = (int)n_out;
    p.x_bytes = n_in > 0 ? ((n_in - 1) * (int64_t)p.ld_x + ((p.Cin + 3) & ~3)) * 4 : 0;
    return conv_dispatch(p, n_in, (hipStream_t)stream);
}

static void params_from_desc(ConvParams &p, const eprecon_conv_desc *d)
{
    p.x = d->x; p.nbr = d->nbr; p.w = d->weight; p.bias = d->bias; p.out = d->out;
    p.K = d->kvol; p.Cin = d->cin; p.Cout = d->cout; p.ld_x = d->ld_x; p.ld_out = d->ld_out;
    p.relu = d->relu; p.accumulate = d->accumulate;
    p.res = d->residual; p.ld_res = d->ld_res; p.bn_partial = d->bn_partial;
    p.in_scale = d->in_scale; p.in_shift = d->in_shift; p.in_relu = d->in_relu;
    p.res_scale = d->res_scale; p.res_shift = d->res_shift; p.res_relu = d->res_relu;
    p.ln = d->ln; p.ln_gamma = d->ln_gamma; p.ln_beta = d->ln_beta; p.ln_eps = d->ln_eps;
    p.ln_post_relu = d->ln_post_relu;
    p.img_h = d->img_h; p.img_w = d->img_w; p.img_maps = d->img_maps;
    p.vox_rank = d->vox_rank; p.gx = d->grid_x; p.gy = d->grid_y; p.gz = d->grid_z; p.wq = d->packed_weight;
    p.wq16 = d->packed_weight16;
    p.ws = d->workspace; p.ws_bytes = d->workspace_bytes;
    p.flex_partial = 1;
    p.bn_acc = d->bn_acc; p.bn_acc_ld = d->bn_acc_ld; p.bn_acc_c0 = d->bn_acc_c0; p.bn_gamma = d->bn_gamma; p.bn_beta = d->bn_beta;
    p.in_acc = d->in_acc; p.in_acc_ld = d->in_acc_ld; p.in_acc_c0 = d->in_acc_c0; p.in_eps = d->in_eps;
}

extern "C" int eprecon_batchnorm_acc_affine_async(const long long *acc, int acc_ld, int acc_c0, int channels, float eps,
                                                  float *scale_out, float *shift_out, void *stream);

static bool bn_acc_family(const ConvParams &p) { return conv3d_kind(p) == 0; }

extern "C" size_t eprecon_bn_acc_words(int ld)
{
    return ld > 0 ? (size_t)epconv::kBnCopies * ld * epconv::kBnWords + (size_t)(2 * ld + 1) / 2 : 0;
}

extern "C" int eprecon_conv_desc_takes_bn_acc(const eprecon_conv_desc *d)
{
    if (!d || d->n_out <= 0) return 0;
    ConvParams p = {};
    params_from_desc(p, d);
    p.n_out = (int)d->n_out;
    return !p.ln && !p.accumulate && bn_acc_family(p) ? 1 : 0;
}

extern "C" int eprecon_conv_desc_async(const eprecon_conv_desc *d, void *stream)
{
    if (!d) return EPRECON_ERR_ARG;
    ConvParams p = {};
    params_from_desc(p, d);
    p.n_out = (int)(d->n_out > 0 && d->n_out <= 0x7fffffff ? d->n_out : 0);
    if (p.bn_acc && (p.bn_acc_ld <= 0 || p.bn_acc_c0 < 0 || p.bn_acc_c0 + p.Cout > p.bn_acc_ld || p.ln || p.accumulate || !bn_acc_family(p)))
        return EPRECON_ERR_ARG;
    if (p.in_acc) {
        if (p.in_scale || p.in_shift || p.in_acc_ld <= 0 || p.in_acc_c0 < 0 || p.in_acc_c0 + p.Cin > p.in_acc_ld) return EPRECON_ERR_ARG;
        if (bn_acc_family(p)) {
            p.in_scale = p.in_shift = reinterpret_cast<const float *>(p.in_acc);
        } else {
            if (!d->in_affine_scratch) return EPRECON_ERR_ARG;
            const int rc = eprecon_batchnorm_acc_affine_async(p.in_acc, p.in_acc_ld, p.in_acc_c0, p.Cin, p.in_eps, d->in_affine_scratch,
                                                              d->in_affine_scratch + p.Cin, stream);
            if (rc != EPRECON_OK) return rc;
            p.in_scale = d->in_affine_scratch;
            p.in_shift = d->in_affine_scratch + p.Cin;
            p.in_acc = nullptr;
        }
    }
    return conv_check_and_run(p, d->n_in, d->n_out, stream);
}

extern "C" size_t eprecon_conv_desc_workspace_bytes(const eprecon_conv_desc *d)
{
    if (!d || d->n_out <= 0 || d->n_out > 0x7fffffff) return 0;
    ConvParams p = {};
    params_from_desc(p, d);
    p.n_out = (int)d->n_out;
    return wide_shape_ok(p) ? wide_workspace_bytes(p) : 0;
}

extern "C" int64_t eprecon_conv_desc_partial_rows(const eprecon_conv_desc *d)
{
    if (!d || d->n_out <= 0) return 0;
    ConvParams p = {};
    params_from_desc(p, d);
    p.n_out = (int)d->n_out;
    int nt, nch;
    int64_t blocks;
    if (const int kind = conv3d_kind(p)) return d3_tiles_kind(p, kind);
    p.x_bytes = d->n_in > 0 ? ((d->n_in - 1) * (int64_t)p.ld_x + ((p.Cin + 3) & ~3)) * 4 : 0;
    if (tile2d16_ok(p)) return tile2d16_partial_rows(p);
    if (p.K == 9 && direct16_ok(p)) return ep::ceil_div(d->n_out, (int64_t)direct16_partial_block_rows(p));
    if (conv2d_tile_ok(p, &nt, &nch, &blocks)) return blocks;
    if (wide_ok(p)) return ep::ceil_div(d->n_out, (int64_t)kWideRows);
    if (splitk_ok(p)) return ep::ceil_div(d->n_out, (int64_t)32);
    if (direct16_ok(p)) return ep::ceil_div(d->n_out, (int64_t)direct16_partial_block_rows(p));
    return ep::ceil_div(d->n_out, (int64_t)kRowsPerBlock);
}

extern "C" int eprecon_sparse_conv_fused_async(const float *x, int64_t n_in, int ld_x, const int32_t *nbr,
                                               int kvol, int64_t n_out, const float *weight, int cin,
                                               int cout, const float *bias, const float *residual,
                                               int ld_res, float *out, int ld_out, int relu,
                                               int accumulate, float *bn_partial, void *stream)
{
    ConvParams p = {};
    p.x = x; p.nbr = nbr; p.w = weight; p.bias = bias; p.out = out;
    p.K = kvol; p.Cin = cin; p.Cout = cout; p.ld_x = ld_x; p.ld_out = ld_out;
    p.relu = relu; p.accumulate = accumulate;
    p.res = residual; p.ld_res = ld_res; p.bn_partial = bn_partial;
    return conv_check_and_run(p, n_in, n_out, stream);
}

extern "C" int eprecon_sparse_conv_async(const float *x, int64_t n_in, int ld_x, const int32_t *nbr,
                                         int kvol, int64_t n_out, const float *weight, int cin,
                                         int cout, const float *bias, float *out, int ld_out,
                                         int relu, int accumulate, void *stream)
{
    return eprecon_sparse_conv_fused_async(x, n_in, ld_x, nbr, kvol, n_out, weight, cin, cout, bias, nullptr, 0,
                                           out, ld_out, relu, accumulate, nullptr, stream);
}
```

### eprecon_amd/csrc/sparse_conv_direct_impl.hpp

```cpp
#pragma once
#include <stdlib.h>

#include <atomic>
#include <type_traits>

#include "common.hpp"
#include "conv_common.hpp"

namespace epconv {
namespace {
using namespace ep;

constexpr int kRT = 2;

#ifndef EP_DIRECT_ABL
#define EP_DIRECT_ABL 0
#endif

__device__ __forceinline__ float relu_nc(float x)
{
    float r;
    asm("v_max_f32 %0, 0, %1" : "=v"(r) : "v"(x));
    return r;
}
// ... 53 lines not shown
        }
    float v[CT][NR];
    bool colok[CT];
#pragma unroll
    for (int t = 0; t < CT; ++t) {
        const int col = 16 * t + l16;
        colok[t] = col < p.Cout;
        const float b = (p.bias && colok[t]) ? p.bias[col] : 0.0f;
        const float rs = (p.res_scale && colok[t]) ? p.res_scale[col] : 1.0f;
        const float rb = (p.res_scale && colok[t]) ? p.res_shift[col] : 0.0f;
#pragma unroll
        for (int r = 0; r < NR; ++r) {
            float val = 0.0f;
            if (colok[t] && orow[r] >= 0) {
                val = acc[r >> 2][t][r & 3] + b;
                if (p.relu) val = fmaxf(val, 0.0f);
                if (p.res) {
                    float rv = p.res[(size_t)orow[r] * p.ld_res + col];
                    if (p.res_scale) {
                        rv = fmaf(rv, rs, rb);
                        if (p.res_relu) rv = fmaxf(rv, 0.0f);
                    }
                    val += rv;
                }
            }
            v[t][r] = val;
        }
    }
    if (p.ln) {
        const float inv_c = 1.0f / (float)p.Cout;
#pragma unroll
        for (int r = 0; r < NR; ++r) {
            float sum = 0.0f;
#pragma unroll
            for (int t = 0; t < CT; ++t) sum += v[t][r];
#pragma unroll
            for (int m = 8; m > 0; m >>= 1) sum += __shfl_xor(sum, m);
            const float mean = sum * inv_c;
            float sq = 0.0f;
#pragma unroll
            for (int t = 0; t < CT; ++t) {
                const float d = colok[t] ? v[t][r] - mean : 0.0f;
                v[t][r] = d;
                sq = fmaf(d, d, sq);
            }
#pragma unroll
            for (int m = 8; m > 0; m >>= 1) sq += __shfl_xor(sq, m);
            const float inv = 1.0f / sqrtf(sq * inv_c + p.ln_eps);
#pragma unroll
            for (int t = 0; t < CT; ++t) {
                const int col = 16 * t + l16;
                float y = fmaf(v[t][r] * inv, (p.ln_gamma && colok[t]) ? p.ln_gamma[col] : 1.0f, (p.ln_beta && colok[t]) ? p.ln_beta[col] : 0.0f);
                if (p.ln_post_relu) y = fmaxf(y, 0.0f);
                v[t][r] = y;
            }
        }
    }
#pragma unroll
    for (int t = 0; t < CT; ++t)
#pragma unroll
        for (int r = 0; r < NR; ++r)
            if (colok[t] && orow[r] >= 0) p.out[(size_t)orow[r] * p.ld_out + 16 * t + l16] = v[t][r];
    if (p.bn_partial || p.bn_acc) {
#pragma unroll
        for (int t = 0; t < CT; ++t) {
            float n = 0.0f, sum = 0.0f;
#pragma unroll
            for (int r = 0; r < NR; ++r)
                if (orow[r] >= 0) { n += 1.0f; sum += v[t][r]; }
            float mean = n > 0.0f ? sum / n : 0.0f, m2 = 0.0f;
#pragma unroll
            for (int r = 0; r < NR; ++r)
                if (orow[r] >= 0) { const float d = v[t][r] - mean; m2 = fmaf(d, d, m2); }
#pragma unroll
            for (int m = 16; m < 64; m <<= 1) {
                const float on = __shfl_xor(n, m), om = __shfl_xor(mean, m), oq = __shfl_xor(m2, m);
                const bool lower = (lane & m) == 0;
                float a_n = lower ? n : on, a_mean = lower ? mean : om, a_m2 = lower ? m2 : oq;
                chan_merge(a_n, a_mean, a_m2, lower ? on : n, lower ? om : mean, lower ? oq : m2);
                n = a_n; mean = a_mean; m2 = a_m2;
            }
            if constexpr (PERWAVE) {
                if (q == 0 && colok[t]) {
                    if (p.bn_partial) {
                        float *dst = p.bn_partial + (size_t)block * 3 * p.Cout + 16 * t + l16;
                        dst[0] = n; dst[p.Cout] = mean; dst[2 * p.Cout] = m2;
                    }
                    if (p.bn_acc) bn_acc_publish(p, 16 * t + l16, block, block == 0, n, mean, m2);
                }
                continue;
            }
            if (q == 0) {
                float *d = sStat + (wave * 3) * 16 * CT + 16 * t + l16;
                d[0] = n; d[16 * CT] = mean; d[2 * 16 * CT] = m2;
            }
        }
        if constexpr (PERWAVE) return;
        __syncthreads();
        if (tid < 16 * CT && tid < p.Cout) {
            float a_n = 0.0f, a_mean = 0.0f, a_m2 = 0.0f;
#pragma unroll
            for (int w = 0; w < kWaves; ++w)
                chan_merge(a_n, a_mean, a_m2, sStat[(w * 3) * 16 * CT + tid], sStat[(w * 3 + 1) * 16 * CT + tid], sStat[(w * 3 + 2) * 16 * CT + tid]);
            if (p.bn_partial) {
                float *dst = p.bn_partial + (size_t)blockIdx.x * 3 * p.Cout + tid;
                dst[0] = a_n; dst[p.Cout] = a_mean; dst[2 * p.Cout] = a_m2;
            }
            if (p.bn_acc) bn_acc_publish(p, tid, (int)blockIdx.x, blockIdx.x == 0, a_n, a_mean, a_m2);
        }
    }
}

__device__ __forceinline__ void tail_to_tile(const f32x4 (&acct)[kRT][2], f32x4 (&dst)[kRT], int lane)
{
    const int l16 = lane & 15, q = lane >> 4;
    const int src = 4 * q + (l16 & 3);
#pragma unroll
    for (int rt = 0; rt < kRT; ++rt)
#pragma unroll
        for (int j = 0; j < 4; ++j) {
            float v0 = acct[rt][0][j], v1 = acct[rt][1][j];
            v0 += __shfl_xor(v0, 16); v1 += __shfl_xor(v1, 16);
            v0 += __shfl_xor(v0, 32); v1 += __shfl_xor(v1, 32);
            const float t0 = __shfl(v0, src), t1 = __shfl(v1, src);
            dst[rt][j] = l16 < 4 ? t0 : (l16 < 8 ? t1 : 0.0f);
        }
}

constexpr int kMapLoads = 14;
__device__ __forceinline__ unsigned stage_map(const ConvParams &p, int row0, int *sNbr, int *sFlag, int tid)
{
    static_assert(kDirectRows == 128 && kRT == 2 && kWaves == 4, "the pass -> (offset, row half) arithmetic below");
    const int total = p.K * kDirectRows;
    const int lane = tid & 63, wave = tid >> 6;
    int jv[kMapLoads];
#pragma unroll
    for (int it = 0; it < kMapLoads; ++it) {
        const int e = tid + it * 256;
        const int k = e >> 7, row = row0 + (e & 127);
        int j = -1;
        if (e < total && row < p.n_out) j = p.nbr ? p.nbr[(size_t)k * p.n_out + row] : row;
        jv[it] = j;
    }
#pragma unroll
    for (int it = 0; it < kMapLoads; ++it) {
        const int e = tid + it * 256;
        if (e < total) sNbr[e] = jv[it];
        const unsigned long long b = __ballot(jv[it] >= 0);
        const int k = 2 * it + (wave >> 1);
        if (lane < 2 && k < p.K) sFlag[k * kWaves + 2 * (wave & 1) + lane] = (lane ? (unsigned)(b >> 32) : (unsigned)b) != 0u;
    }
    __syncthreads();
    const bool mine = lane < p.K && sFlag[lane * kWaves + wave] != 0;
    return (unsigned)__builtin_amdgcn_readfirstlane((int)(unsigned)__ballot(mine));
}

struct LiveCursor {
    unsigned rest;
    int k, part;
    __device__ __forceinline__ explicit LiveCursor(unsigned mask) : rest(mask & (mask - 1u)), k(__builtin_ctz(mask)), part(0) {}
    __device__ __forceinline__ void next(int parts)
    {
        if (part + 1 < parts) ++part;
        else if (rest) { k = __builtin_ctz(rest); rest &= rest - 1u; part = 0; }
    }
};

#ifndef EP_MIX_EXTRA
#define EP_MIX_EXTRA 1
#endif

#ifndef EP_STAGE_CAP
#define EP_STAGE_CAP 3
#endif
constexpr int stage_chunks(int kch) { return kch % 3 == 0 && EP_STAGE_CAP >= 3 ? 3 : (kch % 2 == 0 && EP_STAGE_CAP >= 2 ? 2 : 1); }

template <int CT, int KCH, bool TAIL = false, int G = stage_chunks(KCH), bool BF = false, int MODE = 0>
__global__ __launch_bounds__(256) void spconv_direct16_kernel(ConvParams p)
{
    extern __shared__ __attribute__((aligned(16))) char smem[];
    constexpr int RT = kRT, ROWS = kDirectRows;
    constexpr int CTM = TAIL ? CT - 1 : CT;
    constexpr int CTA = CTM > 0 ? CTM : 1;
    constexpr int PARTS = KCH / G;
    constexpr int cpad = 16 * KCH;
    int *sNbr = reinterpret_cast<int *>(smem);
    float *sStat = reinterpret_cast<float *>(sNbr + p.K * ROWS);
    float *sAff = sStat + kWaves * 3 * 16 * CT;
    int *sFlag = reinterpret_cast<int *>(sAff + 2 * cpad);
    const int tid = threadIdx.x;
// ... 844 lines not shown
```

### eprecon_amd/csrc/spvcnn_forward.hip

```cpp
#include <vector>

#include "common.hpp"

namespace {
using namespace ep;

constexpr int kDirectMaxCout = 64;
constexpr int64_t kK1DirectMinRows = 20000;

enum Slot {
    kStem = 0,
    kS1Down, kS1R1a, kS1R1b, kS1R1d, kS1R2a, kS1R2b,
    kS2Down, kS2R1a, kS2R1b, kS2R1d, kS2R2a, kS2R2b,
    kMlp0,
    kU1Up, kU1R1a, kU1R1b, kU1R1d, kU1R2a, kU1R2b,
    kU2Up, kU2R1a, kU2R1b, kU2R1d, kU2R2a, kU2R2b,
    kMlp1,
    kSlots
};
static_assert(kSlots == EPRECON_SPVCNN_CONVS, "slot table out of step with include/eprecon_hip.h");

struct Rows {
    float *p;
    int64_t n;
// ... 22 lines not shown
                off = free_list[i].off;
                if (free_list[i].bytes == bytes) free_list.erase(free_list.begin() + i);
                else { free_list[i].off += bytes; free_list[i].bytes -= bytes; }
                break;
            }
        if (off == (size_t)-1) {
            off = used;
            used += bytes;
            if (used > peak) peak = used;
        }
        live.push_back(Block{off, bytes});
        if (dry) return reinterpret_cast<void *>(kFakeBase + off);
        if (off + bytes > cap) {
            if (rc == EPRECON_OK) rc = EPRECON_ERR_WORKSPACE;
            return nullptr;
        }
        return base + off;
    }
    void release(const void *p)
    {
        if (!p) return;
        const size_t off = dry ? (size_t)(reinterpret_cast<uintptr_t>(p) - kFakeBase) : (size_t)(static_cast<const char *>(p) - base);
        for (size_t i = 0; i < live.size(); ++i)
            if (live[i].off == off) {
                Block b = live[i];
                live.erase(live.begin() + i);
                size_t k = 0;
                while (k < free_list.size() && free_list[k].off < b.off) ++k;
                free_list.insert(free_list.begin() + k, b);
                if (k + 1 < free_list.size() && free_list[k].off + free_list[k].bytes == free_list[k + 1].off) {
                    free_list[k].bytes += free_list[k + 1].bytes;
                    free_list.erase(free_list.begin() + k + 1);
                }
                if (k > 0 && free_list[k - 1].off + free_list[k - 1].bytes == free_list[k].off) {
                    free_list[k - 1].bytes += free_list[k].bytes;
                    free_list.erase(free_list.begin() + k);
                }
                if (!free_list.empty() && free_list.back().off + free_list.back().bytes == used) {
                    used = free_list.back().off;
                    free_list.pop_back();
                }
                return;
            }
    }
    void release(const Rows &r) { release(r.p); }
    Rows rows(int64_t n, int c, int ld = 0)
    {
        if (ld == 0) ld = (c + 3) & ~3;
        return Rows{static_cast<float *>(alloc((size_t)(n > 0 ? n : 1) * ld * sizeof(float))), n, c, ld};
    }
    static Rows slice(const Rows &r, int c0, int c) { return Rows{r.p ? r.p + c0 : nullptr, r.n, c, r.ld}; }
    void step(int r)
    {
        if (rc == EPRECON_OK && r != EPRECON_OK && r != EPRECON_EMPTY) rc = r;
    }
    bool ok() const { return rc == EPRECON_OK; }

    float *conv(int s, const Rows &x, const int32_t *nbr, int64_t n_out, const Rows &out, const float *in_scale,
                const float *in_shift, int64_t *n_partial)
    {
        const eprecon_spvcnn_conv &w = d->conv[s];
        eprecon_conv_desc c = {};
        c.x = x.p; c.n_in = x.n; c.ld_x = x.ld;
        c.nbr = nbr; c.kvol = w.kvol; c.n_out = n_out;
        c.weight = w.weight; c.cin = w.cin; c.cout = w.cout;
        c.out = out.p; c.ld_out = out.ld;
        c.in_scale = in_scale; c.in_shift = in_shift; c.in_relu = in_scale ? 1 : 0;
        if (!nbr && w.kvol == 1 && w.cout <= kDirectMaxCout && x.n >= kK1DirectMinRows) c.packed_weight16 = w.packed_weight16;
        if (nbr && w.kvol == 27 && w.cout <= kDirectMaxCout) c.packed_weight16 = w.packed_weight16;
        if (nbr && w.kvol == 27) c.packed_weight = w.packed_weight;
        if (x.c != w.cin || out.c != w.cout) {
            step(EPRECON_ERR_ARG);
            return nullptr;
        }
        const size_t need = eprecon_conv_desc_workspace_bytes(&c);
        if (need) {
            c.workspace = alloc(need);
            c.workspace_bytes = need;
        }
        int64_t rows_p = eprecon_conv_desc_partial_rows(&c);
        if (rows_p < 1) rows_p = 1;
        float *partial = static_cast<float *>(alloc((size_t)rows_p * 3 * w.cout * sizeof(float)));
        c.bn_partial = partial;
        *n_partial = rows_p;
        if (!dry && ok() && n_out > 0) step(eprecon_conv_desc_async(&c, stream));
        if (need) release(c.workspace);
        return partial;
    }
    float *affine(int s, const float *partial, int64_t rows_p)
    {
        const eprecon_spvcnn_conv &w = d->conv[s];
        float *aff = static_cast<float *>(alloc((size_t)2 * w.cout * sizeof(float)));
        if (!dry && ok())
            step(eprecon_batchnorm_finalize_affine_async(partial, rows_p, w.cout, d->bn[s].gamma, d->bn[s].beta, d->bn[s].eps, aff,
                                                         aff + w.cout, stream));
        return aff;
    }
    void apply(int s, const Rows &x, const float *partial, int64_t rows_p, const Rows *res, const float *res_aff, const Rows &out)
    {
        const int c = d->conv[s].cout;
        const size_t wsb = eprecon_batchnorm_apply_workspace_bytes(c);
        void *ws = alloc(wsb);
        struct Done { Pass *p; void *ws; ~Done() { p->release(ws); } } done{this, ws};
        if (dry || !ok()) return;
        if (res_aff)
            step(eprecon_batchnorm_apply_partials_res_async(x.p, x.n, c, x.ld, partial, rows_p, d->bn[s].gamma, d->bn[s].beta,
                                                            d->bn[s].eps, res->p, res->ld, res_aff, res_aff + c, 1, out.p, out.ld, ws,
                                                            wsb, stream));
        else
            step(eprecon_batchnorm_apply_partials_async(x.p, x.n, c, x.ld, partial, rows_p, d->bn[s].gamma, d->bn[s].beta,
                                                        d->bn[s].eps, res ? res->p : nullptr, res ? res->ld : 0, 1, out.p, out.ld,
                                                        nullptr, nullptr, ws, wsb, stream));
    }
    Rows basic(int s, const Rows &x, const int32_t *nbr, int64_t n_out, const Rows *out_slot)
    {
        const Rows y = out_slot ? *out_slot : rows(n_out, d->conv[s].cout, d->conv[s].cout);
        int64_t rp = 0;
        const float *p = conv(s, x, nbr, n_out, y, nullptr, nullptr, &rp);
        apply(s, y, p, rp, nullptr, nullptr, y);
        release(p);
        return y;
    }
    Rows residual(int a, bool has_skip, const Rows &x, const int32_t *nbr, const Rows *out_slot)
    {
        const int64_t n = x.n;
        int64_t rp1 = 0, rp2 = 0, rps = 0;
        const Rows y2 = rows(n, d->conv[a + 1].cout, d->conv[a + 1].cout);
        const Rows out = out_slot ? *out_slot : y2;
        const Rows y = rows(n, d->conv[a].cout, d->conv[a].cout);
        const float *p1 = conv(a, x, nbr, n, y, nullptr, nullptr, &rp1);
        const float *aff = affine(a, p1, rp1);
        release(p1);
        const float *p2 = conv(a + 1, y, nbr, n, y2, aff, aff + d->conv[a].cout, &rp2);
        release(y);
        release(aff);
        if (!has_skip) {
            apply(a + 1, y2, p2, rp2, &x, nullptr, out);
        } else {
            const Rows skip = rows(n, d->conv[a + 2].cout, d->conv[a + 2].cout);
            const float *ps = conv(a + 2, x, nullptr, n, skip, nullptr, nullptr, &rps);
            const float *saff = affine(a + 2, ps, rps);
            release(ps);
            apply(a + 1, y2, p2, rp2, &skip, saff, out);
            release(skip);
            release(saff);
        }
        release(p2);
        if (out_slot) release(y2);
        return out;
    }
    void seg_mean(const Rows &feat, const int32_t *offsets, const int32_t *order, const Rows &out)
    {
        if (!dry && ok())
            step(eprecon_segment_mean_async(feat.p, feat.ld, offsets, order, out.n, feat.c, out.p, out.ld, stream));
    }
    void devox(const Rows &vox, const int32_t *idx8, const float *w8, const Rows &out, int accumulate)
    {
        if (!dry && ok())
            step(eprecon_devoxelize_async(vox.p, vox.ld, idx8, w8, out.n, vox.c, out.p, out.ld, accumulate, stream));
    }

    int run()
    {
        const eprecon_spvcnn_forward_desc &D = *d;
        const int *cs = D.cs;
        const int64_t n = D.n, n1 = D.n1, n2 = D.n2, n4 = D.n4;
        const Rows zf{const_cast<float *>(D.feat), n, D.cin, D.ld_feat};
        const Rows cat0 = rows(n1, cs[4] + cs[0], cs[4] + cs[0]), cat1 = rows(n2, cs[3] + cs[1], cs[3] + cs[1]);
        const Rows x0 = rows(n1, D.cin);
        seg_mean(zf, D.offsets1, D.order1, x0);
        const Rows f0_slot = slice(cat0, cs[4], cs[0]);
        const Rows f0 = basic(kStem, x0, D.k1, n1, &f0_slot);
        release(x0);
        const Rows z0 = rows(n, cs[0], cs[0]);
        devox(f0, D.idx8_1, D.weight8_1, z0, 0);
        const Rows x1 = rows(n1, cs[0]);
        seg_mean(z0, D.offsets1, D.order1, x1);
        Rows f = basic(kS1Down, x1, D.down12, n2, nullptr);
        release(x1);
        Rows g = residual(kS1R1a, true, f, D.k2, nullptr);
        release(f);
        const Rows f1_slot = slice(cat1, cs[3], cs[1]);
        const Rows f1 = residual(kS1R2a, false, g, D.k2, &f1_slot);
        release(g);
        f = basic(kS2Down, f1, D.down24, n4, nullptr);
        g = residual(kS2R1a, true, f, D.k4, nullptr);
        release(f);
        const Rows f2 = residual(kS2R2a, false, g, D.k4, nullptr);
        release(g);
        const Rows z1 = rows(n, cs[2], cs[2]);
        basic(kMlp0, z0, nullptr, n, &z1);
        release(z0);
        devox(f2, D.idx8_4, D.weight8_4, z1, 1);
// ... 74 lines not shown
```

### eprecon_amd/dense2d.py

```python
import ctypes
import os

import torch

from . import _lib
from . import sparse as SP


class PixelGrid:
    _cache = {}

    def __init__(self, maps, height, width, device):
        self.maps, self.height, self.width, self.device = maps, height, width, device
        self.n = maps * height * width
        self._nbr = {}

    @classmethod
    def get(cls, maps, height, width, device):
        key = (maps, height, width, str(device))
        g = cls._cache.get(key)
        if g is None:
            g = cls._cache[key] = cls(maps, height, width, device)
        return g

# ... 93 lines not shown
        words = int(_lib.load().eprecon_bn_acc_words(channels))
        return cls(_ARENA.take(words), channels, 0, channels)

    def part(self, a, b):
        return AccSlice(self.block, self.ld, self.c0 + a, b - a)


class Act:
    __slots__ = ("rows", "scale", "shift", "relu", "acc", "eps")

    def __init__(self, rows, scale=None, shift=None, relu=False, acc=None, eps=1e-5):
        self.rows, self.scale, self.shift, self.relu, self.acc, self.eps = rows, scale, shift, relu, acc, eps

    def affine(self):
        if self.acc is not None and self.scale is None:
            a = torch.empty((2, self.acc.c), dtype=torch.float32, device=self.rows.device)
            _lib.check(_lib.load().eprecon_batchnorm_acc_affine_async(
                self.acc.block.data_ptr(), self.acc.ld, self.acc.c0, self.acc.c, float(self.eps), a[0].data_ptr(), a[1].data_ptr(),
                _lib.current_stream()), "eprecon_batchnorm_acc_affine_async")
            self.scale, self.shift = a[0], a[1]
        return self.scale, self.shift


def _dptr(t):
    return None if t is None else t.data_ptr()


def conv_bn_act(conv, bn, x, grid, out=None, aff=None, relu=True, pre_relu=False, residual=None):
    return conv_bn_launch(packed_weight(conv), conv.bias, bn.weight, bn.bias, bn.eps, conv.kernel_size[0], x, grid,
                          out=out, aff=aff, relu=relu, pre_relu=pre_relu, residual=residual)


def conv_bn_launch(w, bias, gamma, beta, eps, k, x, grid, out=None, aff=None, relu=True, pre_relu=False,
                   residual=None):
    lib = _lib.load()
    kvol, cin, cout = w.shape
    rows = x.rows
    n = rows.shape[0]
    dev = rows.device
    assert rows.shape[1] == cin and rows.dtype == torch.float32 and rows.stride(1) == 1
    nbr = grid.kernel_map(k)
    if out is None:
        out = torch.empty((n, cout), dtype=torch.float32, device=dev)
    d = _lib.ConvDesc()
    d.x, d.n_in, d.ld_x = rows.data_ptr(), n, rows.stride(0)
    d.nbr, d.kvol, d.n_out = _dptr(nbr), kvol, n
    d.weight, d.cin, d.cout = w.data_ptr(), cin, cout
    d.bias = _dptr(bias)
    if residual is not None:
        assert residual.rows.shape == (n, cout)
        d.residual, d.ld_res = residual.rows.data_ptr(), residual.rows.stride(0)
        r_scale, r_shift = residual.affine()
        d.res_scale, d.res_shift, d.res_relu = _dptr(r_scale), _dptr(r_shift), int(residual.relu)
    d.out, d.ld_out = out.data_ptr(), out.stride(0)
    d.relu, d.accumulate = int(pre_relu), 0
    if x.acc is not None and x.scale is None:
        assert x.acc.c == cin
        d.in_acc, d.in_acc_ld, d.in_acc_c0, d.in_eps = x.acc.block.data_ptr(), x.acc.ld, x.acc.c0, float(x.eps)
    else:
        d.in_scale, d.in_shift = _dptr(x.scale), _dptr(x.shift)
    d.in_relu = int(x.relu)
    if k == 3:
        d.img_h, d.img_w, d.img_maps = grid.height, grid.width, grid.maps
        if n < DIRECT_2D_MIN_ROWS:
            pq = SP.packed_weight(w)
            d.packed_weight = pq.data_ptr()
        if cout <= SP.DIRECT_MAX_COUT and n >= DIRECT_2D_MIN_ROWS:
            pw = SP.packed_weight16(w)
            d.packed_weight16 = pw.data_ptr()
    elif k == 1 and cout <= SP.DIRECT_MAX_COUT and n >= K1_DIRECT_2D_MIN_ROWS:
        pw = SP.packed_weight16(w)
        d.packed_weight16 = pw.data_ptr()
    if _ARENA is not None and (aff is None or isinstance(aff, AccSlice)) and lib.eprecon_conv_desc_takes_bn_acc(ctypes.byref(d)):
        acc = aff if aff is not None else AccSlice.new(cout)
        assert acc.c == cout
        d.bn_acc, d.bn_acc_ld, d.bn_acc_c0 = acc.block.data_ptr(), acc.ld, acc.c0
        d.bn_gamma, d.bn_beta = _dptr(gamma), _dptr(beta)
        _lib.check(lib.eprecon_conv_desc_async(ctypes.byref(d), _lib.current_stream()), "eprecon_conv_desc_async")
        return Act(out, relu=relu, acc=acc, eps=eps)
    if aff is None:
        a = torch.empty((2, cout), dtype=torch.float32, device=dev)
        aff = (a[0], a[1])
    assert not isinstance(aff, AccSlice), "an accumulator slice was handed to a launch that cannot produce into it"
    partial = torch.empty((lib.eprecon_conv_desc_partial_rows(ctypes.byref(d)), 3, cout), dtype=torch.float32, device=dev)
    d.bn_partial = partial.data_ptr()
    _lib.check(lib.eprecon_conv_desc_async(ctypes.byref(d), _lib.current_stream()), "eprecon_conv_desc_async")
    _lib.check(lib.eprecon_batchnorm_finalize_affine_async(
        partial.data_ptr(), partial.shape[0], cout, _dptr(gamma), _dptr(beta), float(eps),
        aff[0].data_ptr(), aff[1].data_ptr(), _lib.current_stream()), "eprecon_batchnorm_finalize_affine_async")
    return Act(out, aff[0], aff[1], relu)


def materialize(act, out=None):
    if act.scale is None and act.acc is None:
        if out is not None and out.data_ptr() != act.rows.data_ptr():
            out.copy_(act.rows)
            return out
        return act.rows
    rows = act.rows
    n, c = rows.shape
    if out is None:
        out = torch.empty((n, c), dtype=torch.float32, device=rows.device)
    if act.scale is None and c <= 512:
        _lib.check(_lib.load().eprecon_affine_rows_acc_async(
            rows.data_ptr(), n, c, rows.stride(0), act.acc.block.data_ptr(), act.acc.ld, act.acc.c0, float(act.eps), int(act.relu),
            out.data_ptr(), out.stride(0), _lib.current_stream()), "eprecon_affine_rows_acc_async")
        return out
    act.affine()
    _lib.check(_lib.load().eprecon_affine_rows_async(
        rows.data_ptr(), n, c, rows.stride(0), act.scale.data_ptr(), act.shift.data_ptr(), int(act.relu),
        out.data_ptr(), out.stride(0), _lib.current_stream()), "eprecon_affine_rows_async")
    return out


def conv_bn(conv, bn, x, grid, out=None, relu=True, pre_relu=False, pre_residual=None):
    res = Act(pre_residual) if pre_residual is not None else None
    return materialize(conv_bn_act(conv, bn, Act(x), grid, relu=relu, pre_relu=pre_relu, residual=res), out=out)
```

### eprecon_amd/sparse.py

```python
import ctypes

import torch

from . import _lib


import os

def _dense3d_level():
    return int(os.environ.get("EPRECON_CONV_DENSE3D", "2"))


def _ld(t):
    assert t.dim() == 2 and t.stride(1) == 1, "row-major 2-D tensor expected"
    return t.stride(0)


class HashGrid:

    def __init__(self, n, device):
        lib = _lib.load()
        self.capacity = int(lib.eprecon_hash_capacity(int(n)))
        self.mem = torch.empty(int(lib.eprecon_hash_table_bytes(self.capacity)), dtype=torch.uint8,
                               device=device)
# ... 319 lines not shown
        assert ksize == 3
        if self.dims is not None and self.n >= DENSE_MIN_FILL * self.dims[0] * self.dims[1] * self.dims[2] \
                and _dense3d_level() > 0 and self.coords.is_cuda:
            if self._dense is None:
                self._dense = DenseMap(self, self.dims)
            return self._dense
        return self.kernel_map(3)

    @property
    def n(self):
        return self.coords.shape[0]

    @property
    def grid(self):
        if self._grid is None:
            self._grid = HashGrid(self.n, self.coords.device).build(self.coords)
        return self._grid

    def kernel_map(self, ksize=3):
        assert ksize == 3
        if self._k3 is None:
            lib = _lib.load()
            nbr = torch.empty((27, self.n), dtype=torch.int32, device=self.coords.device)
            _lib.check(lib.eprecon_kernel_map_async(_lib.ptr(self.grid.mem), self.grid.capacity,
                                                    _lib.ptr(self.coords), self.n, 3, self.stride,
                                                    _lib.ptr(nbr), _lib.current_stream()),
                       "eprecon_kernel_map_async")
            self._k3 = nbr
        return self._k3

    def downsample(self, pre=None):
        if self._down is None:
            lib = _lib.load()
            q = 2 * self.stride
            uniq, parent, cgrid = pre if pre is not None else unique_coords(self.coords, quantum=q)
            coarse = VoxelSet(uniq, q, grid=cgrid)
            m = coarse.n
            down = torch.empty((8, m), dtype=torch.int32, device=self.coords.device)
            _lib.check(lib.eprecon_kernel_map_async(_lib.ptr(self.grid.mem), self.grid.capacity,
                                                    _lib.ptr(coarse.coords), m, 2, self.stride,
                                                    _lib.ptr(down), _lib.current_stream()),
                       "eprecon_kernel_map_async")
            up = torch.empty((8, self.n), dtype=torch.int32, device=self.coords.device)
            _lib.check(lib.eprecon_transpose_map_async(_lib.ptr(self.coords), self.n, _lib.ptr(parent),
                                                       self.stride, _lib.ptr(up), _lib.current_stream()),
                       "eprecon_transpose_map_async")
            self._down = (coarse, down, up)
        return self._down


def _attach_workspace(desc, device):
    need = int(_lib.load().eprecon_conv_desc_workspace_bytes(ctypes.byref(desc)))
    if not need:
        return None
    ws = _lib.workspace(need, device)
    desc.workspace, desc.workspace_bytes = ws.data_ptr(), ws.numel()
    return ws


def sparse_conv(x, weight, nbr=None, bias=None, out=None, relu=False, accumulate=False):
    lib = _lib.load()
    w_owner = weight
    if weight.dim() == 2:
        weight = weight.unsqueeze(0)
    kvol, cin, cout = weight.shape
    weight = weight.contiguous()
    n_out = x.shape[0] if nbr is None else nbr.shape[1]
    assert x.shape[1] == cin and x.dtype == torch.float32
    if isinstance(nbr, DenseMap) or (kvol == 27 and nbr is not None and x.is_cuda) or \
            (kvol == 1 and nbr is None and x.is_cuda and cout <= DIRECT_MAX_COUT and not accumulate and n_out >= K1_DIRECT_MIN_ROWS):
        return sparse_conv_fused(x, w_owner, nbr, bias, out, relu, None, accumulate)[0]
    if nbr is not None:
        assert nbr.dtype == torch.int32 and nbr.shape[0] == kvol and nbr.is_contiguous()
    if out is None:
        out = torch.empty((n_out, cout), dtype=torch.float32, device=x.device)
    assert out.shape == (n_out, cout)
    _lib.check(lib.eprecon_sparse_conv_async(_lib.ptr(x), x.shape[0], _ld(x), _lib.ptr(nbr), kvol, n_out,
                                             _lib.ptr(weight), cin, cout, _lib.ptr(bias), _lib.ptr(out),
                                             _ld(out), int(relu), int(accumulate), _lib.current_stream()),
               "eprecon_sparse_conv_async")
    return out


def sparse_conv_fused(x, weight, nbr=None, bias=None, out=None, relu=False, residual=None, accumulate=False,
                      bn_partial=False):
    lib = _lib.load()
    w_owner = weight
    if weight.dim() == 2:
        weight = weight.unsqueeze(0)
    kvol, cin, cout = weight.shape
    weight = weight.contiguous()
    n_out = x.shape[0] if nbr is None else nbr.shape[1]
    assert x.shape[1] == cin and x.dtype == torch.float32
    k1_direct = kvol == 1 and nbr is None and x.is_cuda and cout <= DIRECT_MAX_COUT and not accumulate and n_out >= K1_DIRECT_MIN_ROWS
    if isinstance(nbr, DenseMap) or (kvol == 27 and nbr is not None and x.is_cuda) or k1_direct:
        if nbr is not None and not isinstance(nbr, DenseMap):
            assert nbr.dtype == torch.int32 and nbr.shape[0] == kvol and nbr.is_contiguous()
        if out is None:
            out = torch.empty((n_out, cout), dtype=torch.float32, device=x.device)
        assert out.shape == (n_out, cout)
        d = _lib.ConvDesc()
        d.x, d.n_in, d.ld_x = x.data_ptr(), x.shape[0], _ld(x)
        d.kvol, d.n_out = kvol, n_out
        d.weight, d.cin, d.cout = weight.data_ptr(), cin, cout
        d.bias = None if bias is None else bias.data_ptr()
        if residual is not None:
            assert residual.shape == (n_out, cout)
            d.residual, d.ld_res = residual.data_ptr(), _ld(residual)
        d.out, d.ld_out = out.data_ptr(), _ld(out)
        d.relu, d.accumulate = int(relu), int(accumulate)
        keep = _resolve_map(nbr, x, weight, d, accumulate=accumulate, stats=bn_partial, owner=w_owner)
        keep.append(_attach_workspace(d, x.device))
        partial = None
        if bn_partial:
            partial = torch.empty((max(int(lib.eprecon_conv_desc_partial_rows(ctypes.byref(d))), 1), 3, cout),
                                  dtype=torch.float32, device=x.device)
            d.bn_partial = partial.data_ptr()
        _lib.check(lib.eprecon_conv_desc_async(ctypes.byref(d), _lib.current_stream()), "eprecon_conv_desc_async")
        del keep
        return out, partial
    if nbr is not None:
        assert nbr.dtype == torch.int32 and nbr.shape[0] == kvol and nbr.is_contiguous()
    if out is None:
        out = torch.empty((n_out, cout), dtype=torch.float32, device=x.device)
    assert out.shape == (n_out, cout)
    partial = None
    if bn_partial:
        partial = torch.empty(((n_out + 127) // 128, 3, cout), dtype=torch.float32, device=x.device)
    if residual is not None:
        assert residual.shape == (n_out, cout) and residual.dtype == torch.float32
    _lib.check(lib.eprecon_sparse_conv_fused_async(
        _lib.ptr(x), x.shape[0], _ld(x), _lib.ptr(nbr), kvol, n_out, _lib.ptr(weight), cin, cout, _lib.ptr(bias),
        _lib.ptr(residual), _ld(residual) if residual is not None else 0, _lib.ptr(out), _ld(out), int(relu),
        int(accumulate), _lib.ptr(partial), _lib.current_stream()), "eprecon_sparse_conv_fused_async")
    return out, partial


def sparse_conv_ln(x, weight, nbr, bias, ln_weight, ln_bias, ln_eps, out=None, relu=False, residual=None,
                   post_relu=False):
    lib = _lib.load()
    w_owner = weight
    if weight.dim() == 2:
        weight = weight.unsqueeze(0)
    kvol, cin, cout = weight.shape
    weight = weight.contiguous()
    n_out = x.shape[0] if nbr is None else nbr.shape[1]
    assert x.shape[1] == cin and x.dtype == torch.float32 and cout <= 128
    if out is None:
        out = torch.empty((n_out, cout), dtype=torch.float32, device=x.device)
    d = _lib.ConvDesc()
    d.x, d.n_in, d.ld_x = x.data_ptr(), x.shape[0], _ld(x)
    d.kvol, d.n_out = kvol, n_out
    keep = _resolve_map(nbr, x, weight, d, ln=True, owner=w_owner)
    d.weight, d.cin, d.cout = weight.data_ptr(), cin, cout
    d.bias = None if bias is None else bias.data_ptr()
    if residual is not None:
        assert residual.shape == (n_out, cout)
        d.residual, d.ld_res = residual.data_ptr(), _ld(residual)
    d.out, d.ld_out = out.data_ptr(), _ld(out)
    d.relu = int(relu)
    d.ln = 1
    d.ln_gamma = None if ln_weight is None else ln_weight.data_ptr()
    d.ln_beta = None if ln_bias is None else ln_bias.data_ptr()
    d.ln_eps, d.ln_post_relu = float(ln_eps), int(post_relu)
    _lib.check(lib.eprecon_conv_desc_async(ctypes.byref(d), _lib.current_stream()), "eprecon_conv_desc_async")
    return out


def affine_rows(x, scale, shift, residual=None, relu=False, out=None):
    lib = _lib.load()
    n, c = x.shape
    if out is None:
        out = torch.empty((n, c), dtype=torch.float32, device=x.device)
    _lib.check(lib.eprecon_affine_rows_res_async(
        _lib.ptr(x), n, c, _ld(x), _lib.ptr(scale), _lib.ptr(shift), _lib.ptr(residual),
        _ld(residual) if residual is not None else 0, int(relu), _lib.ptr(out), _ld(out), _lib.current_stream()),
        "eprecon_affine_rows_res_async")
    return out


def conv_stats(x, weight, nbr=None, in_affine=None, out=None, bias=None):
    lib = _lib.load()
    w_owner = weight
    if weight.dim() == 2:
        weight = weight.unsqueeze(0)
    kvol, cin, cout = weight.shape
    weight = weight.contiguous()
    n_out = x.shape[0] if nbr is None else nbr.shape[1]
    assert x.shape[1] == cin and x.dtype == torch.float32
    if out is None:
        out = torch.empty((n_out, cout), dtype=torch.float32, device=x.device)
    d = _lib.ConvDesc()
    d.x, d.n_in, d.ld_x = x.data_ptr(), x.shape[0], _ld(x)
    d.kvol, d.n_out = kvol, n_out
    keep = _resolve_map(nbr, x, weight, d, stats=True, owner=w_owner)
    d.weight, d.cin, d.cout = weight.data_ptr(), cin, cout
    d.bias = None if bias is None else bias.data_ptr()
    d.out, d.ld_out = out.data_ptr(), _ld(out)
    if in_affine is not None:
        d.in_scale, d.in_shift, d.in_relu = in_affine[0].data_ptr(), in_affine[1].data_ptr(), int(in_affine[2])
    keep.append(_attach_workspace(d, x.device))
    rows = max(int(lib.eprecon_conv_desc_partial_rows(ctypes.byref(d))), 1)
    partial = torch.empty((rows, 3, cout), dtype=torch.float32, device=x.device)
    d.bn_partial = partial.data_ptr()
    if n_out > 0:
        _lib.check(lib.eprecon_conv_desc_async(ctypes.byref(d), _lib.current_stream()), "eprecon_conv_desc_async")
    return out, partial


def bn_affine(partial, gamma, beta, eps):
    lib = _lib.load()
    c = partial.shape[2]
    aff = torch.empty((2, c), dtype=torch.float32, device=partial.device)
    _lib.check(lib.eprecon_batchnorm_finalize_affine_async(
        partial.data_ptr(), partial.shape[0], c, _lib.ptr(gamma), _lib.ptr(beta), float(eps), aff[0].data_ptr(),
        aff[1].data_ptr(), _lib.current_stream()), "eprecon_batchnorm_finalize_affine_async")
    return aff[0], aff[1]


def batchnorm_apply_partials(x, partial, gamma=None, beta=None, eps=1e-5, residual=None, relu=False, out=None,
                             res_affine=None):
    lib = _lib.load()
    n, c = x.shape
    assert partial.shape[1:] == (3, c) and partial.is_contiguous()
    if out is None:
        out = torch.empty((n, c), dtype=torch.float32, device=x.device)
    ws = torch.empty((lib.eprecon_batchnorm_apply_workspace_bytes(c),), dtype=torch.uint8, device=x.device)
    if res_affine is not None:
        _lib.check(lib.eprecon_batchnorm_apply_partials_res_async(
            _lib.ptr(x), n, c, _ld(x), _lib.ptr(partial), partial.shape[0], _lib.ptr(gamma), _lib.ptr(beta), float(eps),
            _lib.ptr(residual), _ld(residual), _lib.ptr(res_affine[0]), _lib.ptr(res_affine[1]), int(relu), _lib.ptr(out),
            _ld(out), _lib.ptr(ws), ws.numel(), _lib.current_stream()), "eprecon_batchnorm_apply_partials_res_async")
        return out
    _lib.check(lib.eprecon_batchnorm_apply_partials_async(
        _lib.ptr(x), n, c, _ld(x), _lib.ptr(partial), partial.shape[0], _lib.ptr(gamma), _lib.ptr(beta),
        float(eps), _lib.ptr(residual), _ld(residual) if residual is not None else 0, int(relu), _lib.ptr(out),
        _ld(out), None, None, _lib.ptr(ws), ws.numel(), _lib.current_stream()),
        "eprecon_batchnorm_apply_partials_async")
    return out


def batchnorm_train(x, gamma=None, beta=None, eps=1e-5, residual=None, relu=False, out=None):
    lib = _lib.load()
    n, c = x.shape
    if out is None:
        out = torch.empty((n, c), dtype=torch.float32, device=x.device)
    ws = _lib.workspace(lib.eprecon_batchnorm_workspace_bytes(n, c), x.device)
    _lib.check(lib.eprecon_batchnorm_train_async(
        _lib.ptr(x), n, c, _ld(x), _lib.ptr(gamma), _lib.ptr(beta), float(eps), _lib.ptr(residual),
        _ld(residual) if residual is not None else 0, int(relu), _lib.ptr(out), _ld(out), None, None,
        _lib.ptr(ws), ws.numel(), _lib.current_stream()), "eprecon_batchnorm_train_async")
    return out


def rowwise_layernorm(x, gamma=None, beta=None, eps=1e-5, residual=None, pre_relu=False, post_relu=False,
                      out=None):
    lib = _lib.load()
    n, c = x.shape
    if out is None:
        out = torch.empty((n, c), dtype=torch.float32, device=x.device)
    _lib.check(lib.eprecon_rowwise_layernorm_async(
        _lib.ptr(x), n, c, _ld(x), _lib.ptr(residual), _ld(residual) if residual is not None else 0,
        _lib.ptr(gamma), _lib.ptr(beta), float(eps), int(pre_relu), int(post_relu), _lib.ptr(out),
        _ld(out), _lib.current_stream()), "eprecon_rowwise_layernorm_async")
    return out


def _pack_mlp_weight(wt):
    k, m = wt.shape
    kc, mt = (k + 15) // 16, (m + 15) // 16
    w = torch.zeros((16 * kc, 16 * mt), dtype=torch.float32, device=wt.device)
    w[:k, :m] = wt
    return w.view(kc, 4, 4, mt, 16).permute(3, 0, 1, 4, 2).contiguous().view(-1)


def _pad16(v, n=None):
    n = v.shape[0] if n is None else n
    out = torch.zeros(((n + 15) // 16 * 16,), dtype=torch.float32, device=v.device)
    out[:v.shape[0]] = v
    return out


def mlp4x_supported(channels, out_channels):
    return bool(_lib.load().eprecon_mlp4x_supported(int(channels), int(out_channels)))


def pack_mlp4x(mod):
    params = (mod.linear1.weight, mod.linear1.bias, mod.norm1.weight, mod.norm1.bias, mod.linear2.weight, mod.linear2.bias,
              mod.norm2.weight, mod.norm2.bias, mod.linear3.weight, mod.linear3.bias)
    tag = tuple((p_._version, p_.data_ptr()) for p_ in params)
    hit = getattr(mod, "_eprecon_packed", None)
    if hit is not None and hit[0] == tag:
        return hit[1]
    with torch.no_grad():
        parts = {"w1": _pack_mlp_weight(mod.linear1.weight.t()), "b1": _pad16(mod.linear1.bias), "g1": _pad16(mod.norm1.weight),
                 "be1": _pad16(mod.norm1.bias), "w2": _pack_mlp_weight(mod.linear2.weight.t()), "b2": _pad16(mod.linear2.bias),
                 "g2": _pad16(mod.norm2.weight), "be2": _pad16(mod.norm2.bias), "w3": _pack_mlp_weight(mod.linear3.weight.t()),
                 "b3": _pad16(mod.linear3.bias)}
        flat = torch.cat([v for v in parts.values()])
        views, off = {}, 0
        for name, v in parts.items():
            views[name] = flat[off:off + v.numel()]
            off += v.numel()
    mod._eprecon_packed = (tag, views)
    return views


def mlp4x(mods, x, outs=None):
    lib = _lib.load()
    m0 = mods[0]
    c, cout = m0.linear1.in_features, m0.linear3.out_features
    n = x.shape[0]
    assert x.dtype == torch.float32 and x.stride(1) == 1 and x.shape[1] >= c and 1 <= len(mods) <= 2
    d = _lib.Mlp4xDesc()
    d.x, d.ld_x, d.n = x.data_ptr(), x.stride(0), n
    d.channels, d.out_channels, d.heads, d.residual = c, cout, len(mods), int(m0.use_residual)
    d.eps1, d.eps2 = float(m0.norm1.eps), float(m0.norm2.eps)
    if outs is None:
# ... 13 lines not shown
```

### include/eprecon_hip.h

```cpp
#ifndef EPRECON_HIP_H
#define EPRECON_HIP_H

#include <stddef.h>
#include <stdint.h>

#ifdef __cplusplus
extern "C" {
#endif

#define EPRECON_OK 0
#define EPRECON_EMPTY 1
#define EPRECON_ERR_ARG (-1)
#define EPRECON_ERR_WORKSPACE (-2)
#define EPRECON_ERR_UNSUPPORTED (-3)
#define EPRECON_ERR_HIP_BASE (-1000)

#define EPRECON_ABI_VERSION 1
int eprecon_abi_version(void);
const char *eprecon_build_arch(void);

#define EPRECON_BP_MEAN 0
#define EPRECON_BP_MEAN_DEPTH 1
#define EPRECON_BP_VARIANCE 2

// ... 8 lines not shown
                               const float *krcam, int n_views, int channels, int height,
                               int width, int min_view, int mode, float *out_feats,
                               float *out_mean, int32_t *out_coords, float *count,
                               float *out_grid, uint8_t *out_mask, int32_t *n_valid_dev,
                               void *workspace, size_t workspace_bytes, void *stream);

int eprecon_back_project(const int32_t *coords, int64_t n, const float *origin, int batch,
                         float voxel_size, const float *feats, int feats_layout,
                         const float *krcam, int n_views, int channels, int height, int width,
                         int min_view, int mode, int min_valid_per_batch, float *out_feats,
                         float *out_mean, int32_t *out_coords, float *count, float *out_grid,
                         uint8_t *out_mask, int32_t *n_valid_dev, int32_t *n_valid_host,
                         void *workspace, size_t workspace_bytes, void *stream);

int eprecon_profile_enable(int on);
float eprecon_profile_gather_ms(void);
const char *eprecon_profile_gather_kernel(void);

int eprecon_profile_conv_arm(int kvol, int cin, int cout, int64_t min_rows);
float eprecon_profile_conv_ms(int64_t *rows_out, const char **kernel_out);
int64_t eprecon_profile_conv_pairs(void);
int64_t eprecon_profile_conv_executed_pairs(void);
const char *eprecon_profile_last_conv_kernel(void);
int eprecon_profile_mark_async(int id, void *stream);

int eprecon_nchw_to_nhwc_async(const float *in, float *out, int maps, int channels, int hw,
                               void *stream);
typedef struct eprecon_views_desc {
    const float *src[3][16];
    float *dst[3];
    int32_t channels[3]; int32_t hw[3];
    int32_t levels; int32_t n_views;
} eprecon_views_desc;
int eprecon_views_to_rows_async(const eprecon_views_desc *desc, void *stream);

uint32_t eprecon_hash_capacity(int64_t n);
size_t eprecon_hash_table_bytes(uint32_t capacity);
int eprecon_hash_build_async(const int32_t *coords, int64_t n, int quantum, void *table,
                             uint32_t capacity, void *stream);
int eprecon_hash_build_dn_async(const int32_t *coords, int64_t n_cap, const int32_t *n_dev, int quantum, void *table,
                                uint32_t capacity, void *stream);
int eprecon_hash_query_async(const void *table, uint32_t capacity, const int32_t *queries, int64_t m,
                             int quantum, int32_t *out_index, void *stream);
int eprecon_hash_status(const void *table, void *stream);

size_t eprecon_unique_workspace_bytes(int64_t n);
int eprecon_exclusive_scan_async(const int32_t *in, int64_t n, int32_t *out, int32_t *total, int32_t *scratch, void *stream);
int eprecon_unique_coords_async(const int32_t *coords, int64_t n, int quantum, void *table,
                                uint32_t capacity, int32_t *inverse, int32_t *unique_coords,
                                int32_t *n_unique_dev, void *workspace, size_t workspace_bytes,
                                void *stream);

int eprecon_unique_coords_dn_async(const int32_t *coords, int64_t n_cap, const int32_t *n_dev, int quantum, void *table,
                                   uint32_t capacity, int32_t *inverse, int32_t *unique_coords, int32_t *n_unique_dev,
                                   void *workspace, size_t workspace_bytes, void *stream);
int eprecon_unique_hierarchy_dn_async(const int32_t *coords, int64_t n_cap, const int32_t *n_dev, int levels, void *const *tables,
                                      const uint32_t *capacities, int32_t *const *inverse, int32_t *const *unique_coords,
                                      int32_t *summary, void *workspace, size_t workspace_bytes, void *stream);

int eprecon_kernel_map_self_async(const void *table, uint32_t capacity, const int32_t *coords, int64_t n, int stride, int32_t *nbr,
                                  void *stream);
int eprecon_kernel_map_async(const void *table, uint32_t capacity, const int32_t *coords, int64_t n,
                             int ksize, int stride, int32_t *nbr, void *stream);
int eprecon_transpose_map_async(const int32_t *fine_coords, int64_t n, const int32_t *parent,
                                int fine_stride, int32_t *up_map, void *stream);
int eprecon_sparse_conv_async(const float *x, int64_t n_in, int ld_x, const int32_t *nbr, int kvol,
                              int64_t n_out, const float *weight, int cin, int cout, const float *bias,
                              float *out, int ld_out, int relu, int accumulate, void *stream);
size_t eprecon_conv_bn_partial_bytes(int64_t n_out, int cout);
int eprecon_sparse_conv_fused_async(const float *x, int64_t n_in, int ld_x, const int32_t *nbr, int kvol,
                                    int64_t n_out, const float *weight, int cin, int cout,
                                    const float *bias, const float *residual, int ld_res, float *out,
                                    int ld_out, int relu, int accumulate, float *bn_partial, void *stream);
typedef struct eprecon_conv_desc {
    const float *x; int64_t n_in; int ld_x;
    const int32_t *nbr; int kvol; int64_t n_out;
    const float *weight; int cin; int cout;
    const float *bias;
    const float *residual; int ld_res;
    float *out; int ld_out;
    int relu; int accumulate;
    const float *in_scale; const float *in_shift; int in_relu;
    const float *res_scale; const float *res_shift; int res_relu;
    float *bn_partial;
    int ln; const float *ln_gamma; const float *ln_beta; float ln_eps; int ln_post_relu;
    int img_h; int img_w; int img_maps;
    const int32_t *vox_rank; int grid_x; int grid_y; int grid_z;
    const float *packed_weight;
    const float *packed_weight16;
    void *workspace; size_t workspace_bytes;
    long long *bn_acc; int bn_acc_ld; int bn_acc_c0; const float *bn_gamma; const float *bn_beta;
    const long long *in_acc; int in_acc_ld; int in_acc_c0; float in_eps; float *in_affine_scratch;
} eprecon_conv_desc;
size_t eprecon_bn_acc_words(int ld);
int eprecon_conv_desc_takes_bn_acc(const eprecon_conv_desc *desc);
int eprecon_batchnorm_acc_affine_async(const long long *acc, int acc_ld, int acc_c0, int channels, float eps, float *scale_out,
                                       float *shift_out, void *stream);
int eprecon_affine_rows_acc_async(const float *x, int64_t n, int channels, int ld_x, const long long *acc, int acc_ld, int acc_c0,
                                  float eps, int relu, float *out, int ld_out, void *stream);
int eprecon_conv_desc_async(const eprecon_conv_desc *desc, void *stream);
size_t eprecon_conv_desc_workspace_bytes(const eprecon_conv_desc *desc);
int64_t eprecon_conv_desc_partial_rows(const eprecon_conv_desc *desc);
int eprecon_batchnorm_finalize_affine_async(const float *partial, int64_t nblk, int channels, const float *gamma,
                                            const float *beta, float eps, float *scale_out, float *shift_out,
                                            void *stream);
int eprecon_affine_rows_async(const float *x, int64_t n, int channels, int ld_x, const float *scale,
                              const float *shift, int relu, float *out, int ld_out, void *stream);
int eprecon_affine_rows_res_async(const float *x, int64_t n, int channels, int ld_x, const float *scale,
                                  const float *shift, const float *residual, int ld_res, int relu, float *out,
                                  int ld_out, void *stream);
int eprecon_pixel_map_async(int maps, int height, int width, int ksize, int32_t *nbr, void *stream);
int eprecon_grid_rank_async(const int32_t *coords, int64_t n, int stride, int grid_x, int grid_y, int grid_z, int32_t *rank,
                            void *stream);
size_t eprecon_conv_pack_weight_floats(int kvol, int cin, int cout);
int eprecon_conv_pack_weight_async(const float *weight, int kvol, int cin, int cout, float *packed, void *stream);
size_t eprecon_conv_pack_weight16_floats(int kvol, int cin, int cout);
int eprecon_conv_pack_weight16_async(const float *weight, int kvol, int cin, int cout, float *packed, void *stream);
typedef struct eprecon_pack_job {
    const float *weight; float *packed;
    int32_t kvol; int32_t cin; int32_t cout; int32_t kind;
} eprecon_pack_job;
int eprecon_conv_pack_many_async(const eprecon_pack_job *jobs, int njobs, void *stream);

size_t eprecon_batchnorm_workspace_bytes(int64_t n, int channels);
int eprecon_batchnorm_train_async(const float *x, int64_t n, int channels, int ld_x, const float *gamma,
                                  const float *beta, float eps, const float *residual, int ld_res,
                                  int relu, float *out, int ld_out, float *mean_out, float *var_out,
                                  void *workspace, size_t workspace_bytes, void *stream);
size_t eprecon_batchnorm_apply_workspace_bytes(int channels);
int eprecon_batchnorm_apply_partials_async(const float *x, int64_t n, int channels, int ld_x,
                                           const float *partial, int64_t nblk, const float *gamma,
                                           const float *beta, float eps, const float *residual,
                                           int ld_res, int relu, float *out, int ld_out, float *mean_out,
                                           float *var_out, void *workspace, size_t workspace_bytes,
                                           void *stream);
int eprecon_batchnorm_apply_partials_res_async(const float *x, int64_t n, int channels, int ld_x, const float *partial,
                                               int64_t nblk, const float *gamma, const float *beta, float eps,
                                               const float *residual, int ld_res, const float *res_scale,
                                               const float *res_shift, int relu, float *out, int ld_out, void *workspace,
                                               size_t workspace_bytes, void *stream);
int eprecon_rowwise_layernorm_async(const float *x, int64_t n, int channels, int ld_x,
                                    const float *residual, int ld_res, const float *gamma,
                                    const float *beta, float eps, int pre_relu, int post_relu,
                                    float *out, int ld_out, void *stream);

size_t eprecon_init_select_workspace_bytes(int batch, int dim);
int eprecon_init_select_async(const float *logit, const int32_t *coords, int64_t n, float threshold,
                              int batch, int dim, int cell, int32_t *out_coords, int32_t *n_out_dev,
                              void *workspace, size_t workspace_bytes, void *stream);
size_t eprecon_sparsify_workspace_bytes(int64_t n);
int eprecon_sparsify_async(const float *occ, int ld_occ, float threshold, const unsigned char *target,
                           const int32_t *coords, const float *tsdf, int ld_tsdf, const float *feat_all, int ld_feat,
                           int c_all, int c_feat, int64_t n, int batch, int32_t *out_coords, float *out_tsdf,
                           float *out_occ, float *out_all, float *out_feat, int32_t *counts, void *workspace,
                           size_t workspace_bytes, void *stream);
int eprecon_upsample_async(const float *feat, int ld_feat, const int32_t *coords, int64_t n, int channels,
                           int interval, float *up_feat, int32_t *up_coords, void *stream);

int eprecon_aligned_coords_async(const int32_t *coords, int64_t n, const float *origin, int batch,
                                 float voxel_size, const float *world_to_aligned_camera, float *out_xyzb,
                                 void *stream);
int eprecon_point_quantize_async(const float *points_xyzb, int64_t n, float resolution, float *scaled_xyzb,
                                 int32_t *voxel_bxyz, void *stream);
int eprecon_spvcnn_points_dn_async(const int32_t *src_coords, int64_t cap_src, const int32_t *n_src_dev, int children,
                                   int interval, const float *origin, int batch, float voxel_size,
                                   const float *world_to_aligned_camera, float resolution, int32_t *up_coords, float *r_coords,
                                   float *scaled_xyzb, int32_t *voxel_bxyz, int32_t *n_points_dev, void *stream);
int eprecon_point_quantize_dn_async(const float *points_xyzb, int64_t n_cap, const int32_t *n_dev, float resolution,
                                    float *scaled_xyzb, int32_t *voxel_bxyz, void *stream);
size_t eprecon_segment_workspace_bytes(int64_t n, int64_t m);
int eprecon_segment_lists_async(const int32_t *idx, int64_t n, int64_t m, int32_t *offsets, int32_t *order,
                                void *workspace, size_t workspace_bytes, void *stream);
int eprecon_segment_mean_async(const float *feat, int ld_feat, const int32_t *offsets, const int32_t *order,
                               int64_t m, int channels, float *out, int ld_out, void *stream);
int eprecon_sphash_async(const int32_t *coords, int64_t n, int64_t *out_hash, void *stream);
size_t eprecon_sphash_order_workspace_bytes(int64_t n);
int eprecon_sphash_order_async(const int32_t *coords, int64_t n, int32_t *perm_out, int32_t *rank_out, void *workspace,
                               size_t workspace_bytes, void *stream);
int eprecon_remap_index_async(const int32_t *idx, int64_t n, const int32_t *rank_old, const int32_t *perm_new,
                              int64_t m_new, int32_t *out, void *stream);
int eprecon_trilinear_map_async(const void *table, uint32_t capacity, const float *points_xyzb, int64_t n,
                                int stride, int32_t *idx8, float *weight8, void *stream);
int eprecon_devoxelize_async(const float *voxel_feat, int ld_feat, const int32_t *idx8, const float *weight8,
                             int64_t n, int channels, float *out, int ld_out, int accumulate, void *stream);

#define EPRECON_GATE_SIGMOID 1
#define EPRECON_GATE_SIGMOID_MUL 2
#define EPRECON_GATE_GRU_MIX 3
int eprecon_devoxelize_gate_async(const float *voxel_feat, int ld_feat, const int32_t *idx8, const float *weight8,
                                  int64_t n, int channels, const float *skip, int ld_skip, int mode, const float *h,
                                  int ld_h, const float *zgate, int ld_z, float *out, int ld_out, void *stream);

int eprecon_devoxelize_gate_tail_async(const float *voxel_feat, int ld_feat, const int32_t *idx8, const float *weight8,
                                       int64_t n, int channels, const float *skip, int ld_skip, int mode, const float *h,
                                       int ld_h, const float *zgate, int ld_z, float *out, int ld_out, const float *tail_src,
                                       int ld_tail_src, float *tail_dst, int ld_tail_dst, int tail_channels, void *stream);

size_t eprecon_fbv_union_workspace_bytes(int dim);
int eprecon_fbv_union_async(const int32_t *cur_coords, const float *cur_feat, int64_t n_cur, int ld_cur,
                            const int32_t *glob_coords, const float *glob_feat, int64_t n_glob, int ld_glob,
                            int channels, int dim, int interval, int activity_mode,
                            const int32_t *relative_origin_host, int32_t *updated, int32_t *src_cur, int32_t *src_glob, uint8_t *glob_valid,
                            int32_t *n_out_dev, void *workspace, size_t workspace_bytes, void *stream);
int eprecon_gather_rows_async(const float *feat, int ld_feat, const int32_t *src, int64_t n, int channels,
                              float fill, float *out, int ld_out, void *stream);

int eprecon_map_create(int channels, void **out_handle);
int eprecon_map_destroy(void *handle);
int eprecon_map_reset(void *handle);
int64_t eprecon_map_size(const void *handle);
int eprecon_map_channels(const void *handle);
int eprecon_map_export_async(const void *handle, int32_t *coords_out, float *feats_out, void *stream);
int eprecon_map_import_async(void *handle, const int32_t *coords, const float *feats, int64_t n, void *stream);
int eprecon_map_crop_union(void *handle, const int32_t *cur_coords, const float *cur_feat, int64_t n_cur, int ld_cur,
                           int dim, int interval, int activity_mode, const int32_t *relative_origin_host,
                           int32_t *updated, int32_t *src_cur, int32_t *src_glob, int64_t *counts_host, void *stream);
int eprecon_map_gather_async(const void *handle, const int32_t *src_glob, int64_t n, int col0, int channels, float fill,
                             float *out, int ld_out, void *stream);
int eprecon_map_update_async(void *handle, const int32_t *updated, int64_t n, const float *values, int ld_values,
                             void *stream);
// ... 236 lines not shown
```

Baseline: 703.9.

## Store BatchNorm partial summaries channel-major and adapt finalize unroll to block count

Batch-norm partial statistics (n, mean, m2) move from a row-major [block][3][C] layout to a channel-major [3][C][ld] layout, so the per-channel finalize kernels read contiguous block entries and coalesce. All producers (conv epilogues, stats kernel) write through a new strided store helper, and the ABI, descriptor and Python wrappers gain a leading-dimension argument. The finalize kernels are templated on an unroll factor chosen from the block count. In exchange, the producer-side writes become strided across blocks, so those stores coalesce less well.

Result: no change. 717.0 (median of 6 runs) (+1.9%).

```diff
diff --git a/eprecon_amd/_lib.py b/eprecon_amd/_lib.py
--- a/eprecon_amd/_lib.py
+++ b/eprecon_amd/_lib.py
@@ -49,14 +49,14 @@
     "eprecon_batchnorm_acc_affine_async": (_i, [_vp, _i, _i, _i, _f, _vp, _vp, _vp]),
     "eprecon_affine_rows_acc_async": (_i, [_vp, _i64, _i, _i, _vp, _i, _i, _f, _i, _vp, _i, _vp]),
     "eprecon_affine_rows_res_async": (_i, [_vp, _i64, _i, _i, _vp, _vp, _vp, _i, _i, _vp, _i, _vp]),
-    "eprecon_batchnorm_finalize_affine_async": (_i, [_vp, _i64, _i, _vp, _vp, _f, _vp, _vp, _vp]),
+    "eprecon_batchnorm_finalize_affine_async": (_i, [_vp, _i64, _i64, _i, _vp, _vp, _f, _vp, _vp, _vp]),
     "eprecon_affine_rows_async": (_i, [_vp, _i64, _i, _i, _vp, _vp, _i, _vp, _i, _vp]),
     "eprecon_pixel_map_async": (_i, [_i, _i, _i, _i, _vp, _vp]),
     "eprecon_batchnorm_apply_workspace_bytes": (_sz, [_i]),
-    "eprecon_batchnorm_apply_partials_async": (_i, [_vp, _i64, _i, _i, _vp, _i64, _vp, _vp, _f, _vp, _i, _i, _vp, _i,
+    "eprecon_batchnorm_apply_partials_async": (_i, [_vp, _i64, _i, _i, _vp, _i64, _i64, _vp, _vp, _f, _vp, _i, _i, _vp, _i,
                                                     _vp, _vp, _vp, _sz, _vp]),
-    "eprecon_batchnorm_apply_partials_res_async": (_i, [_vp, _i64, _i, _i, _vp, _i64, _vp, _vp, _f, _vp, _i, _vp, _vp, _i, _vp,
-                                                        _i, _vp, _sz, _vp]),
+    "eprecon_batchnorm_apply_partials_res_async": (_i, [_vp, _i64, _i, _i, _vp, _i64, _i64, _vp, _vp, _f, _vp, _i, _vp, _vp, _i,
+                                                        _vp, _i, _vp, _sz, _vp]),
     "eprecon_batchnorm_workspace_bytes": (_sz, [_i64, _i]),
     "eprecon_batchnorm_train_async": (_i, [_vp, _i64, _i, _i, _vp, _vp, _f, _vp, _i, _i, _vp, _i, _vp, _vp,
                                            _vp, _sz, _vp]),
@@ -237,7 +237,7 @@
                 ("relu", ctypes.c_int), ("accumulate", ctypes.c_int),
                 ("in_scale", ctypes.c_void_p), ("in_shift", ctypes.c_void_p), ("in_relu", ctypes.c_int),
                 ("res_scale", ctypes.c_void_p), ("res_shift", ctypes.c_void_p), ("res_relu", ctypes.c_int),
-                ("bn_partial", ctypes.c_void_p),
+                ("bn_partial", ctypes.c_void_p), ("bn_ld", ctypes.c_int),
                 ("ln", ctypes.c_int), ("ln_gamma", ctypes.c_void_p), ("ln_beta", ctypes.c_void_p),
                 ("ln_eps", ctypes.c_float), ("ln_post_relu", ctypes.c_int),
                 ("img_h", ctypes.c_int), ("img_w", ctypes.c_int), ("img_maps", ctypes.c_int),
diff --git a/eprecon_amd/csrc/conv_common.hpp b/eprecon_amd/csrc/conv_common.hpp
--- a/eprecon_amd/csrc/conv_common.hpp
+++ b/eprecon_amd/csrc/conv_common.hpp
@@ -16,6 +16,7 @@
     const float *res;
     int ld_res;
     float *bn_partial;
+    int bn_ld;
     const float *in_scale, *in_shift;
     int in_relu;
     const float *res_scale, *res_shift;
@@ -138,6 +139,13 @@
     n_a = n;
 }
 
+__device__ __forceinline__ void bn_partial_store(const ConvParams &p, int row, int col, float n, float mean, float m2)
+{
+    const size_t plane = (size_t)p.Cout * p.bn_ld;
+    float *dst = p.bn_partial + (size_t)col * p.bn_ld + row;
+    dst[0] = n; dst[plane] = mean; dst[2 * plane] = m2;
+}
+
 template <int CT, bool ACC = false>
 __device__ __forceinline__ void tile16_epilogue(const ConvParams &p, const f32x4 (&acc)[CT], const int (&orow)[4], float *sStat,
                                                 int partial_row)
@@ -236,10 +244,7 @@
 #pragma unroll
             for (int w = 0; w < kWaves; ++w)
                 chan_merge(a_n, a_mean, a_m2, sStat[(w * 3) * 16 * CT + tid], sStat[(w * 3 + 1) * 16 * CT + tid], sStat[(w * 3 + 2) * 16 * CT + tid]);
-            if (p.bn_partial) {
-                float *dst = p.bn_partial + (size_t)partial_row * 3 * p.Cout + tid;
-                dst[0] = a_n; dst[p.Cout] = a_mean; dst[2 * p.Cout] = a_m2;
-            }
+            if (p.bn_partial) bn_partial_store(p, partial_row, tid, a_n, a_mean, a_m2);
             if (ACC && p.bn_acc) bn_acc_publish(p, tid, partial_row, partial_row == 0, a_n, a_mean, a_m2);
         }
     }
diff --git a/eprecon_amd/csrc/norm.hip b/eprecon_amd/csrc/norm.hip
--- a/eprecon_amd/csrc/norm.hip
+++ b/eprecon_amd/csrc/norm.hip
@@ -62,30 +62,46 @@
         __syncthreads();
     }
     if (tid < C) {
-        float *p = partial + (size_t)blockIdx.x * 3 * C;
-        p[tid] = sN[tid]; p[C + tid] = sMean[tid]; p[2 * C + tid] = sM2[tid];
-    }
-}
-
-__global__ __launch_bounds__(256) void bn_finalize_kernel(const float *partial, int nblk, int C, float *mean_out,
+        const size_t plane = (size_t)C * gridDim.x;
+        float *p = partial + (size_t)tid * gridDim.x + blockIdx.x;
+        p[0] = sN[tid]; p[plane] = sMean[tid]; p[2 * plane] = sM2[tid];
+    }
+}
+
+template <int NU>
+__device__ __forceinline__ void bn_merge_rows(const float *partial, int nblk, int64_t ld, int C, int c, int tid, float &a_n,
+                                              float &a_mean, float &a_m2)
+{
+    const float *pn = partial + (size_t)c * ld, *pm = pn + (size_t)C * ld, *pq = pm + (size_t)C * ld;
+    for (int b = tid; b < nblk; b += NU * 256) {
+        float vn[NU], vm[NU], vq[NU];
+#pragma unroll
+        for (int u = 0; u < NU; ++u) {
+            const int bb = b + u * 256;
+            const bool ok = bb < nblk;
+            vn[u] = ok ? pn[bb] : 0.0f;
+            vm[u] = ok ? pm[bb] : 0.0f;
+            vq[u] = ok ? pq[bb] : 0.0f;
+        }
+#pragma unroll
+        for (int u = 0; u < NU; ++u) chan_merge(a_n, a_mean, a_m2, vn[u], vm[u], vq[u]);
+    }
+}
+
+inline int bn_finalize_nu(int64_t nblk)
+{
+    const int64_t need = (nblk + 255) / 256;
+    return need <= 1 ? 1 : need <= 2 ? 2 : need <= 4 ? 4 : need <= 8 ? 8 : 16;
+}
+
+template <int NU>
+__global__ __launch_bounds__(256) void bn_finalize_kernel(const float *partial, int nblk, int64_t ld, int C, float *mean_out,
                                                           float *var_out)
 {
     __shared__ float sN[256], sMean[256], sM2[256];
     const int c = blockIdx.x, tid = threadIdx.x;
     float a_n = 0.0f, a_mean = 0.0f, a_m2 = 0.0f;
-    for (int b = tid; b < nblk; b += 4 * 256) {
-        float vn[4], vm[4], vq[4];
-#pragma unroll
-        for (int u = 0; u < 4; ++u) {
-            const int bb = b + u * 256;
-            const float *p = partial + (size_t)(bb < nblk ? bb : b) * 3 * C;
-            vn[u] = bb < nblk ? p[c] : 0.0f;
-            vm[u] = p[C + c];
-            vq[u] = p[2 * C + c];
-        }
-#pragma unroll
-        for (int u = 0; u < 4; ++u) chan_merge(a_n, a_mean, a_m2, vn[u], vm[u], vq[u]);
-    }
+    bn_merge_rows<NU>(partial, nblk, ld, C, c, tid, a_n, a_mean, a_m2);
     sN[tid] = a_n; sMean[tid] = a_mean; sM2[tid] = a_m2;
     __syncthreads();
     for (int s = 128; s > 0; s >>= 1) {
@@ -102,27 +118,16 @@
     }
 }
 
-__global__ __launch_bounds__(256) void bn_finalize_affine_kernel(const float *partial, int nblk, int C, const float *gamma,
-                                                                 const float *beta, float eps, float *scale_out,
-                                                                 float *shift_out)
+template <int NU>
+__global__ __launch_bounds__(256) void bn_finalize_affine_kernel(const float *partial, int nblk, int64_t ld, int C,
+                                                                 const float *gamma, const float *beta, float eps,
+                                                                 float *scale_out, float *shift_out)
 {
     __shared__ float sN[4], sMean[4], sM2[4];
     const int c = blockIdx.x, tid = threadIdx.x;
     const float g_c = gamma ? gamma[c] : 1.0f, b_c = beta ? beta[c] : 0.0f;
     float a_n = 0.0f, a_mean = 0.0f, a_m2 = 0.0f;
-    for (int b = tid; b < nblk; b += 4 * 256) {
-        float vn[4], vm[4], vq[4];
-#pragma unroll
-        for (int u = 0; u < 4; ++u) {
-            const int bb = b + u * 256;
-            const float *p = partial + (size_t)(bb < nblk ? bb : b) * 3 * C;
-            vn[u] = bb < nblk ? p[c] : 0.0f;
-            vm[u] = p[C + c];
-            vq[u] = p[2 * C + c];
-        }
-#pragma unroll
-        for (int u = 0; u < 4; ++u) chan_merge(a_n, a_mean, a_m2, vn[u], vm[u], vq[u]);
-    }
+    bn_merge_rows<NU>(partial, nblk, ld, C, c, tid, a_n, a_mean, a_m2);
     const int lane = tid & 63;
 #pragma unroll
     for (int m = 1; m < 64; m <<= 1) {
@@ -258,12 +263,17 @@
     out[(size_t)r * ld_out + c] = v;
 }
 
-int bn_finalize_apply(const float *x, int64_t n, int channels, int ld_x, const float *partial, int nblk,
+int bn_finalize_apply(const float *x, int64_t n, int channels, int ld_x, const float *partial, int nblk, int64_t ld,
                       const float *gamma, const float *beta, float eps, const float *residual, int ld_res,
                       int relu, float *out, int ld_out, float *mean, float *var, hipStream_t st,
                       const float *res_scale = nullptr, const float *res_shift = nullptr)
 {
-    hipLaunchKernelGGL(bn_finalize_kernel, dim3(channels), dim3(256), 0, st, partial, nblk, channels, mean, var);
+    switch (bn_finalize_nu(nblk)) {
+#define EP_FINALIZE(NU) \
+    case NU: hipLaunchKernelGGL(bn_finalize_kernel<NU>, dim3(channels), dim3(256), 0, st, partial, nblk, ld, channels, mean, var); break
+        EP_FINALIZE(1); EP_FINALIZE(2); EP_FINALIZE(4); EP_FINALIZE(8); EP_FINALIZE(16);
+#undef EP_FINALIZE
+    }
     EP_LAUNCH_CHECK();
     const size_t total = (size_t)n * channels;
     hipLaunchKernelGGL(bn_apply_kernel, dim3((unsigned)ceil_div((int64_t)total, 256)), dim3(256), 0, st, x,
@@ -306,7 +316,7 @@
     float *var = var_out ? var_out : reinterpret_cast<float *>(ws);
     hipLaunchKernelGGL(bn_stats_kernel, dim3(nblk), dim3(256), 0, st, x, (int)n, channels, ld_x, partial);
     EP_LAUNCH_CHECK();
-    return bn_finalize_apply(x, n, channels, ld_x, partial, nblk, gamma, beta, eps, residual, ld_res, relu, out,
+    return bn_finalize_apply(x, n, channels, ld_x, partial, nblk, nblk, gamma, beta, eps, residual, ld_res, relu, out,
                              ld_out, mean, var, st);
 }
 
@@ -316,13 +326,13 @@
 }
 
 int eprecon_batchnorm_apply_partials_async(const float *x, int64_t n, int channels, int ld_x,
-                                           const float *partial, int64_t nblk, const float *gamma,
+                                           const float *partial, int64_t nblk, int64_t ld, const float *gamma,
                                            const float *beta, float eps, const float *residual,
                                            int ld_res, int relu, float *out, int ld_out, float *mean_out,
                                            float *var_out, void *workspace, size_t workspace_bytes,
                                            void *stream)
 {
-    if (!x || !out || !partial || n < 0 || nblk <= 0 || nblk > 0x7fffffff || channels <= 0 || ld_x < channels ||
+    if (!x || !out || !partial || n < 0 || nblk <= 0 || nblk > 0x7fffffff || ld < nblk || channels <= 0 || ld_x < channels ||
         ld_out < channels || !workspace)
         return EPRECON_ERR_ARG;
     if (workspace_bytes < eprecon_batchnorm_apply_workspace_bytes(channels)) return EPRECON_ERR_WORKSPACE;
@@ -331,17 +341,17 @@
     float *mean = mean_out ? mean_out : reinterpret_cast<float *>(ws);
     ws += align_up((size_t)channels * sizeof(float), 256);
     float *var = var_out ? var_out : reinterpret_cast<float *>(ws);
-    return bn_finalize_apply(x, n, channels, ld_x, partial, (int)nblk, gamma, beta, eps, residual, ld_res, relu,
+    return bn_finalize_apply(x, n, channels, ld_x, partial, (int)nblk, ld, gamma, beta, eps, residual, ld_res, relu,
                              out, ld_out, mean, var, (hipStream_t)stream);
 }
 
 int eprecon_batchnorm_apply_partials_res_async(const float *x, int64_t n, int channels, int ld_x, const float *partial,
-                                               int64_t nblk, const float *gamma, const float *beta, float eps,
+                                               int64_t nblk, int64_t ld, const float *gamma, const float *beta, float eps,
                                                const float *residual, int ld_res, const float *res_scale,
                                                const float *res_shift, int relu, float *out, int ld_out, void *workspace,
                                                size_t workspace_bytes, void *stream)
 {
-    if (!x || !out || !partial || !residual || !res_scale || !res_shift || n < 0 || nblk <= 0 || nblk > 0x7fffffff ||
+    if (!x || !out || !partial || !residual || !res_scale || !res_shift || n < 0 || nblk <= 0 || nblk > 0x7fffffff || ld < nblk ||
         channels <= 0 || ld_x < channels || ld_out < channels || ld_res < channels || !workspace)
         return EPRECON_ERR_ARG;
     if (workspace_bytes < eprecon_batchnorm_apply_workspace_bytes(channels)) return EPRECON_ERR_WORKSPACE;
@@ -349,17 +359,25 @@
     char *ws = reinterpret_cast<char *>(workspace);
     float *mean = reinterpret_cast<float *>(ws);
     float *var = reinterpret_cast<float *>(ws + align_up((size_t)channels * sizeof(float), 256));
-    return bn_finalize_apply(x, n, channels, ld_x, partial, (int)nblk, gamma, beta, eps, residual, ld_res, relu, out, ld_out,
+    return bn_finalize_apply(x, n, channels, ld_x, partial, (int)nblk, ld, gamma, beta, eps, residual, ld_res, relu, out, ld_out,
                              mean, var, (hipStream_t)stream, res_scale, res_shift);
 }
 
-int eprecon_batchnorm_finalize_affine_async(const float *partial, int64_t nblk, int channels, const float *gamma,
+int eprecon_batchnorm_finalize_affine_async(const float *partial, int64_t nblk, int64_t ld, int channels, const float *gamma,
                                             const float *beta, float eps, float *scale_out, float *shift_out,
                                             void *stream)
 {
-    if (!partial || !scale_out || !shift_out || nblk <= 0 || nblk > 0x7fffffff || channels <= 0) return EPRECON_ERR_ARG;
-    hipLaunchKernelGGL(bn_finalize_affine_kernel, dim3(channels), dim3(256), 0, (hipStream_t)stream, partial, (int)nblk,
-                       channels, gamma, beta, eps, scale_out, shift_out);
+    if (!partial || !scale_out || !shift_out || nblk <= 0 || nblk > 0x7fffffff || ld < nblk || channels <= 0) return EPRECON_ERR_ARG;
+    hipStream_t st = (hipStream_t)stream;
+    switch (bn_finalize_nu(nblk)) {
+#define EP_FINALIZE(NU)                                                                                                            \
+    case NU:                                                                                                                       \
+        hipLaunchKernelGGL(bn_finalize_affine_kernel<NU>, dim3(channels), dim3(256), 0, st, partial, (int)nblk, ld, channels, gamma, \
+                           beta, eps, scale_out, shift_out);                                                                         \
+        break
+        EP_FINALIZE(1); EP_FINALIZE(2); EP_FINALIZE(4); EP_FINALIZE(8); EP_FINALIZE(16);
+#undef EP_FINALIZE
+    }
     EP_LAUNCH_CHECK();
     return EPRECON_OK;
 }
diff --git a/eprecon_amd/csrc/sparse_conv.hip b/eprecon_amd/csrc/sparse_conv.hip
--- a/eprecon_amd/csrc/sparse_conv.hip
+++ b/eprecon_amd/csrc/sparse_conv.hip
@@ -199,10 +199,7 @@
             for (int w = 0; w < kWaves; ++w)
                 chan_merge(a_n, a_mean, a_m2, sStat[(w * 3) * TN + tid], sStat[(w * 3 + 1) * TN + tid],
                            sStat[(w * 3 + 2) * TN + tid]);
-            if (!ACC || p.bn_partial) {
-                float *dst = p.bn_partial + (size_t)partial_row * 3 * p.Cout + col0 + tid;
-                dst[0] = a_n; dst[p.Cout] = a_mean; dst[2 * p.Cout] = a_m2;
-            }
+            if (!ACC || p.bn_partial) bn_partial_store(p, partial_row, col0 + tid, a_n, a_mean, a_m2);
             if (ACC && p.bn_acc) bn_acc_publish(p, col0 + tid, partial_row, partial_row == 0, a_n, a_mean, a_m2);
         }
     }
@@ -867,10 +864,7 @@
         sWn[e] = c < p.Cin ? p.w[((size_t)k * p.Cin + c) * p.Cout] : 0.0f;
     }
     if (!d3_stage_halo<NCH, WV>(p, x0, y0, z0, sX, tid, p.debug)) {
-        if (p.bn_partial && tid == 0) {
-            float *dst = p.bn_partial + (size_t)tile * 3 * p.Cout;
-            dst[0] = 0.0f; dst[p.Cout] = 0.0f; dst[2 * p.Cout] = 0.0f;
-        }
+        if (p.bn_partial && tid == 0) bn_partial_store(p, tile, 0, 0.0f, 0.0f, 0.0f);
         return;
     }
     const int v = tid >> 1, part = tid & 1;
@@ -921,8 +915,7 @@
         if (tid == 0) {
             float a_n = 0.0f, a_mean = 0.0f, a_m2 = 0.0f;
             for (int w = 0; w < kWaves; ++w) chan_merge(a_n, a_mean, a_m2, sRed[w * 3], sRed[w * 3 + 1], sRed[w * 3 + 2]);
-            float *dst = p.bn_partial + (size_t)tile * 3 * p.Cout;
-            dst[0] = a_n; dst[p.Cout] = a_mean; dst[2 * p.Cout] = a_m2;
+            bn_partial_store(p, tile, 0, a_n, a_mean, a_m2);
         }
     }
 }
@@ -994,10 +987,7 @@
     float *sStat = sX;
 
     if (!d3_stage_ranks<NCH, kD16X, 256>(p, x0, y0, z0, sX, tid)) {
-        if (p.bn_partial && tid < 16 * CT && tid < p.Cout) {
-            float *dst = p.bn_partial + (size_t)tile * 3 * p.Cout + tid;
-            dst[0] = 0.0f; dst[p.Cout] = 0.0f; dst[2 * p.Cout] = 0.0f;
-        }
+        if (p.bn_partial && tid < 16 * CT && tid < p.Cout) bn_partial_store(p, tile, tid, 0.0f, 0.0f, 0.0f);
         return;
     }
     const int wx = wave >> 1, wy = 2 * (wave & 1);
@@ -2093,7 +2083,7 @@
     p.x = d->x; p.nbr = d->nbr; p.w = d->weight; p.bias = d->bias; p.out = d->out;
     p.K = d->kvol; p.Cin = d->cin; p.Cout = d->cout; p.ld_x = d->ld_x; p.ld_out = d->ld_out;
     p.relu = d->relu; p.accumulate = d->accumulate;
-    p.res = d->residual; p.ld_res = d->ld_res; p.bn_partial = d->bn_partial;
+    p.res = d->residual; p.ld_res = d->ld_res; p.bn_partial = d->bn_partial; p.bn_ld = d->bn_ld;
     p.in_scale = d->in_scale; p.in_shift = d->in_shift; p.in_relu = d->in_relu;
     p.res_scale = d->res_scale; p.res_shift = d->res_shift; p.res_relu = d->res_relu;
     p.ln = d->ln; p.ln_gamma = d->ln_gamma; p.ln_beta = d->ln_beta; p.ln_eps = d->ln_eps;
@@ -2126,12 +2116,19 @@
     return !p.ln && !p.accumulate && bn_acc_family(p) ? 1 : 0;
 }
 
+extern "C" int64_t eprecon_conv_desc_partial_rows(const eprecon_conv_desc *d);
+
 extern "C" int eprecon_conv_desc_async(const eprecon_conv_desc *d, void *stream)
 {
     if (!d) return EPRECON_ERR_ARG;
     ConvParams p = {};
     params_from_desc(p, d);
     p.n_out = (int)(d->n_out > 0 && d->n_out <= 0x7fffffff ? d->n_out : 0);
+    if (p.bn_partial) {
+        const int64_t rows = eprecon_conv_desc_partial_rows(d);
+        if (p.bn_ld == 0) p.bn_ld = (int)(rows > 0 ? rows : 1);
+        if (p.bn_ld < rows) return EPRECON_ERR_ARG;
+    }
     if (p.bn_acc && (p.bn_acc_ld <= 0 || p.bn_acc_c0 < 0 || p.bn_acc_c0 + p.Cout > p.bn_acc_ld || p.ln || p.accumulate || !bn_acc_family(p)))
         return EPRECON_ERR_ARG;
     if (p.in_acc) {
@@ -2190,6 +2187,7 @@
     p.K = kvol; p.Cin = cin; p.Cout = cout; p.ld_x = ld_x; p.ld_out = ld_out;
     p.relu = relu; p.accumulate = accumulate;
     p.res = residual; p.ld_res = ld_res; p.bn_partial = bn_partial;
+    p.bn_ld = (int)ep::ceil_div(n_out > 0 ? n_out : 1, (int64_t)kRowsPerBlock);
     return conv_check_and_run(p, n_in, n_out, stream);
 }
 
diff --git a/eprecon_amd/csrc/sparse_conv_direct_impl.hpp b/eprecon_amd/csrc/sparse_conv_direct_impl.hpp
--- a/eprecon_amd/csrc/sparse_conv_direct_impl.hpp
+++ b/eprecon_amd/csrc/sparse_conv_direct_impl.hpp
@@ -159,10 +159,7 @@
             }
             if constexpr (PERWAVE) {
                 if (q == 0 && colok[t]) {
-                    if (p.bn_partial) {
-                        float *dst = p.bn_partial + (size_t)block * 3 * p.Cout + 16 * t + l16;
-                        dst[0] = n; dst[p.Cout] = mean; dst[2 * p.Cout] = m2;
-                    }
+                    if (p.bn_partial) bn_partial_store(p, block, 16 * t + l16, n, mean, m2);
                     if (p.bn_acc) bn_acc_publish(p, 16 * t + l16, block, block == 0, n, mean, m2);
                 }
                 continue;
@@ -179,10 +176,7 @@
 #pragma unroll
             for (int w = 0; w < kWaves; ++w)
                 chan_merge(a_n, a_mean, a_m2, sStat[(w * 3) * 16 * CT + tid], sStat[(w * 3 + 1) * 16 * CT + tid], sStat[(w * 3 + 2) * 16 * CT + tid]);
-            if (p.bn_partial) {
-                float *dst = p.bn_partial + (size_t)blockIdx.x * 3 * p.Cout + tid;
-                dst[0] = a_n; dst[p.Cout] = a_mean; dst[2 * p.Cout] = a_m2;
-            }
+            if (p.bn_partial) bn_partial_store(p, (int)blockIdx.x, tid, a_n, a_mean, a_m2);
             if (p.bn_acc) bn_acc_publish(p, tid, (int)blockIdx.x, blockIdx.x == 0, a_n, a_mean, a_m2);
         }
     }
diff --git a/eprecon_amd/csrc/spvcnn_forward.hip b/eprecon_amd/csrc/spvcnn_forward.hip
--- a/eprecon_amd/csrc/spvcnn_forward.hip
+++ b/eprecon_amd/csrc/spvcnn_forward.hip
@@ -128,6 +128,7 @@
         if (rows_p < 1) rows_p = 1;
         float *partial = static_cast<float *>(alloc((size_t)rows_p * 3 * w.cout * sizeof(float)));
         c.bn_partial = partial;
+        c.bn_ld = (int)rows_p;
         *n_partial = rows_p;
         if (!dry && ok() && n_out > 0) step(eprecon_conv_desc_async(&c, stream));
         if (need) release(c.workspace);
@@ -138,7 +139,7 @@
         const eprecon_spvcnn_conv &w = d->conv[s];
         float *aff = static_cast<float *>(alloc((size_t)2 * w.cout * sizeof(float)));
         if (!dry && ok())
-            step(eprecon_batchnorm_finalize_affine_async(partial, rows_p, w.cout, d->bn[s].gamma, d->bn[s].beta, d->bn[s].eps, aff,
+            step(eprecon_batchnorm_finalize_affine_async(partial, rows_p, rows_p, w.cout, d->bn[s].gamma, d->bn[s].beta, d->bn[s].eps, aff,
                                                          aff + w.cout, stream));
         return aff;
     }
@@ -150,11 +151,11 @@
         struct Done { Pass *p; void *ws; ~Done() { p->release(ws); } } done{this, ws};
         if (dry || !ok()) return;
         if (res_aff)
-            step(eprecon_batchnorm_apply_partials_res_async(x.p, x.n, c, x.ld, partial, rows_p, d->bn[s].gamma, d->bn[s].beta,
+            step(eprecon_batchnorm_apply_partials_res_async(x.p, x.n, c, x.ld, partial, rows_p, rows_p, d->bn[s].gamma, d->bn[s].beta,
                                                             d->bn[s].eps, res->p, res->ld, res_aff, res_aff + c, 1, out.p, out.ld, ws,
                                                             wsb, stream));
         else
-            step(eprecon_batchnorm_apply_partials_async(x.p, x.n, c, x.ld, partial, rows_p, d->bn[s].gamma, d->bn[s].beta,
+            step(eprecon_batchnorm_apply_partials_async(x.p, x.n, c, x.ld, partial, rows_p, rows_p, d->bn[s].gamma, d->bn[s].beta,
                                                         d->bn[s].eps, res ? res->p : nullptr, res ? res->ld : 0, 1, out.p, out.ld,
                                                         nullptr, nullptr, ws, wsb, stream));
     }
diff --git a/eprecon_amd/dense2d.py b/eprecon_amd/dense2d.py
--- a/eprecon_amd/dense2d.py
+++ b/eprecon_amd/dense2d.py
@@ -199,11 +199,12 @@
         a = torch.empty((2, cout), dtype=torch.float32, device=dev)
         aff = (a[0], a[1])
     assert not isinstance(aff, AccSlice), "an accumulator slice was handed to a launch that cannot produce into it"
-    partial = torch.empty((lib.eprecon_conv_desc_partial_rows(ctypes.byref(d)), 3, cout), dtype=torch.float32, device=dev)
-    d.bn_partial = partial.data_ptr()
+    partial = SP.bn_summaries(lib.eprecon_conv_desc_partial_rows(ctypes.byref(d)), cout, dev)
+    nblk, ld = SP.summary_layout(partial)
+    d.bn_partial, d.bn_ld = partial.data_ptr(), ld
     _lib.check(lib.eprecon_conv_desc_async(ctypes.byref(d), _lib.current_stream()), "eprecon_conv_desc_async")
     _lib.check(lib.eprecon_batchnorm_finalize_affine_async(
-        partial.data_ptr(), partial.shape[0], cout, _dptr(gamma), _dptr(beta), float(eps),
+        partial.data_ptr(), nblk, ld, cout, _dptr(gamma), _dptr(beta), float(eps),
         aff[0].data_ptr(), aff[1].data_ptr(), _lib.current_stream()), "eprecon_batchnorm_finalize_affine_async")
     return Act(out, aff[0], aff[1], relu)
 
diff --git a/eprecon_amd/sparse.py b/eprecon_amd/sparse.py
--- a/eprecon_amd/sparse.py
+++ b/eprecon_amd/sparse.py
@@ -425,6 +425,18 @@
     return out
 
 
+def bn_summaries(rows, cout, device):
+    return torch.empty((3, cout, max(int(rows), 1)), dtype=torch.float32, device=device).permute(2, 0, 1)
+
+
+def summary_layout(partial):
+    nblk, three, c = partial.shape
+    s0, s1, s2 = partial.stride()
+    assert three == 3 and partial.dtype == torch.float32 and s0 == 1 and s2 >= nblk and s1 == c * s2, \
+        "BatchNorm summaries must be the channel-major view bn_summaries() returns"
+    return nblk, s2
+
+
 def sparse_conv_fused(x, weight, nbr=None, bias=None, out=None, relu=False, residual=None, accumulate=False,
                       bn_partial=False):
     lib = _lib.load()
@@ -456,9 +468,8 @@
         keep.append(_attach_workspace(d, x.device))
         partial = None
         if bn_partial:
-            partial = torch.empty((max(int(lib.eprecon_conv_desc_partial_rows(ctypes.byref(d))), 1), 3, cout),
-                                  dtype=torch.float32, device=x.device)
-            d.bn_partial = partial.data_ptr()
+            partial = bn_summaries(lib.eprecon_conv_desc_partial_rows(ctypes.byref(d)), cout, x.device)
+            d.bn_partial, d.bn_ld = partial.data_ptr(), summary_layout(partial)[1]
         _lib.check(lib.eprecon_conv_desc_async(ctypes.byref(d), _lib.current_stream()), "eprecon_conv_desc_async")
         del keep
         return out, partial
@@ -469,7 +480,7 @@
     assert out.shape == (n_out, cout)
     partial = None
     if bn_partial:
-        partial = torch.empty(((n_out + 127) // 128, 3, cout), dtype=torch.float32, device=x.device)
+        partial = bn_summaries((n_out + 127) // 128, cout, x.device)
     if residual is not None:
         assert residual.shape == (n_out, cout) and residual.dtype == torch.float32
     _lib.check(lib.eprecon_sparse_conv_fused_async(
@@ -543,9 +554,8 @@
     if in_affine is not None:
         d.in_scale, d.in_shift, d.in_relu = in_affine[0].data_ptr(), in_affine[1].data_ptr(), int(in_affine[2])
     keep.append(_attach_workspace(d, x.device))
-    rows = max(int(lib.eprecon_conv_desc_partial_rows(ctypes.byref(d))), 1)
-    partial = torch.empty((rows, 3, cout), dtype=torch.float32, device=x.device)
-    d.bn_partial = partial.data_ptr()
+    partial = bn_summaries(lib.eprecon_conv_desc_partial_rows(ctypes.byref(d)), cout, x.device)
+    d.bn_partial, d.bn_ld = partial.data_ptr(), summary_layout(partial)[1]
     if n_out > 0:
         _lib.check(lib.eprecon_conv_desc_async(ctypes.byref(d), _lib.current_stream()), "eprecon_conv_desc_async")
     return out, partial
@@ -554,9 +564,10 @@
 def bn_affine(partial, gamma, beta, eps):
     lib = _lib.load()
     c = partial.shape[2]
+    nblk, ld = summary_layout(partial)
     aff = torch.empty((2, c), dtype=torch.float32, device=partial.device)
     _lib.check(lib.eprecon_batchnorm_finalize_affine_async(
-        partial.data_ptr(), partial.shape[0], c, _lib.ptr(gamma), _lib.ptr(beta), float(eps), aff[0].data_ptr(),
+        partial.data_ptr(), nblk, ld, c, _lib.ptr(gamma), _lib.ptr(beta), float(eps), aff[0].data_ptr(),
         aff[1].data_ptr(), _lib.current_stream()), "eprecon_batchnorm_finalize_affine_async")
     return aff[0], aff[1]
 
@@ -565,18 +576,19 @@
                              res_affine=None):
     lib = _lib.load()
     n, c = x.shape
-    assert partial.shape[1:] == (3, c) and partial.is_contiguous()
+    assert partial.shape[1:] == (3, c)
+    nblk, ld = summary_layout(partial)
     if out is None:
         out = torch.empty((n, c), dtype=torch.float32, device=x.device)
     ws = torch.empty((lib.eprecon_batchnorm_apply_workspace_bytes(c),), dtype=torch.uint8, device=x.device)
     if res_affine is not None:
         _lib.check(lib.eprecon_batchnorm_apply_partials_res_async(
-            _lib.ptr(x), n, c, _ld(x), _lib.ptr(partial), partial.shape[0], _lib.ptr(gamma), _lib.ptr(beta), float(eps),
+            _lib.ptr(x), n, c, _ld(x), _lib.ptr(partial), nblk, ld, _lib.ptr(gamma), _lib.ptr(beta), float(eps),
             _lib.ptr(residual), _ld(residual), _lib.ptr(res_affine[0]), _lib.ptr(res_affine[1]), int(relu), _lib.ptr(out),
             _ld(out), _lib.ptr(ws), ws.numel(), _lib.current_stream()), "eprecon_batchnorm_apply_partials_res_async")
         return out
     _lib.check(lib.eprecon_batchnorm_apply_partials_async(
-        _lib.ptr(x), n, c, _ld(x), _lib.ptr(partial), partial.shape[0], _lib.ptr(gamma), _lib.ptr(beta),
+        _lib.ptr(x), n, c, _ld(x), _lib.ptr(partial), nblk, ld, _lib.ptr(gamma), _lib.ptr(beta),
         float(eps), _lib.ptr(residual), _ld(residual) if residual is not None else 0, int(relu), _lib.ptr(out),
         _ld(out), None, None, _lib.ptr(ws), ws.numel(), _lib.current_stream()),
         "eprecon_batchnorm_apply_partials_async")
diff --git a/include/eprecon_hip.h b/include/eprecon_hip.h
--- a/include/eprecon_hip.h
+++ b/include/eprecon_hip.h
@@ -114,7 +114,7 @@
     int relu; int accumulate;
     const float *in_scale; const float *in_shift; int in_relu;
     const float *res_scale; const float *res_shift; int res_relu;
-    float *bn_partial;
+    float *bn_partial; int bn_ld;
     int ln; const float *ln_gamma; const float *ln_beta; float ln_eps; int ln_post_relu;
     int img_h; int img_w; int img_maps;
     const int32_t *vox_rank; int grid_x; int grid_y; int grid_z;
@@ -133,7 +133,7 @@
 int eprecon_conv_desc_async(const eprecon_conv_desc *desc, void *stream);
 size_t eprecon_conv_desc_workspace_bytes(const eprecon_conv_desc *desc);
 int64_t eprecon_conv_desc_partial_rows(const eprecon_conv_desc *desc);
-int eprecon_batchnorm_finalize_affine_async(const float *partial, int64_t nblk, int channels, const float *gamma,
+int eprecon_batchnorm_finalize_affine_async(const float *partial, int64_t nblk, int64_t ld, int channels, const float *gamma,
                                             const float *beta, float eps, float *scale_out, float *shift_out,
                                             void *stream);
 int eprecon_affine_rows_async(const float *x, int64_t n, int channels, int ld_x, const float *scale,
@@ -161,13 +161,13 @@
                                   void *workspace, size_t workspace_bytes, void *stream);
 size_t eprecon_batchnorm_apply_workspace_bytes(int channels);
 int eprecon_batchnorm_apply_partials_async(const float *x, int64_t n, int channels, int ld_x,
-                                           const float *partial, int64_t nblk, const float *gamma,
+                                           const float *partial, int64_t nblk, int64_t ld, const float *gamma,
                                            const float *beta, float eps, const float *residual,
                                            int ld_res, int relu, float *out, int ld_out, float *mean_out,
                                            float *var_out, void *workspace, size_t workspace_bytes,
                                            void *stream);
 int eprecon_batchnorm_apply_partials_res_async(const float *x, int64_t n, int channels, int ld_x, const float *partial,
-                                               int64_t nblk, const float *gamma, const float *beta, float eps,
+                                               int64_t nblk, int64_t ld, const float *gamma, const float *beta, float eps,
                                                const float *residual, int ld_res, const float *res_scale,
                                                const float *res_shift, int relu, float *out, int ld_out, void *workspace,
                                                size_t workspace_bytes, void *stream);
```
